# aszepieniec/stark-brainfuck

Hardware: AMD Instinct MI355X
Metric: goldilocks_ntt_field_elements_per_sec (higher is better)
Workload: dtype u64 (mod 2^64-2^32+1)

## Files before the change

include/bfstark.h:

```cpp
#ifndef BFSTARK_H
#define BFSTARK_H

#include <stddef.h>
#include <stdint.h>

#ifdef __cplusplus
extern "C" {
#endif

enum {
    BFS_OK = 0,
    BFS_ERR_NOT_POW2 = 1,
    BFS_ERR_NOT_ROOT = 2,
    BFS_ERR_NOT_PRIMITIVE = 3,
    BFS_ERR_TOO_MANY_COEFFS = 4,
    BFS_ERR_ZERO_IN_BATCH_INVERSE = 5,
    BFS_ERR_BAD_ARG = 6,
    BFS_ERR_HIP = 7,
    BFS_ERR_LENGTH = 8,
    BFS_ERR_TOO_MANY_INDICES = 9
};

int bfs_version(void);
const char* bfs_last_error(void);
int bfs_device_count(int* count);
int bfs_set_device(int device);
int bfs_malloc(void** d_ptr, size_t bytes);
int bfs_free(void* d_ptr);
int bfs_malloc_async(void** d_ptr, size_t bytes, void* stream);
int bfs_free_async(void* d_ptr, void* stream);
int bfs_pool_trim(void);
int bfs_pool_stats(size_t* live_bytes, size_t* cached_bytes);
int bfs_host_alloc(void** h_ptr, size_t bytes);
int bfs_host_free(void* h_ptr);
int bfs_memcpy_h2d(void* d_dst, const void* h_src, size_t bytes, void* stream);
int bfs_memcpy_d2h(void* h_dst, const void* d_src, size_t bytes, void* stream);
int bfs_memcpy_d2d(void* d_dst, const void* d_src, size_t bytes, void* stream);
int bfs_memset(void* d_dst, int value, size_t bytes, void* stream);
int bfs_stream_synchronize(void* stream);
int bfs_stream_create(void** stream);
int bfs_stream_destroy(void* stream);
int bfs_event_create(void** event);
int bfs_event_destroy(void* event);
int bfs_event_record(void* event, void* stream);
int bfs_event_elapsed_ms(void* start, void* stop, float* ms);

uint64_t bfs_gl_primitive_root(uint32_t log_n);
uint64_t bfs_gl_mul(uint64_t a, uint64_t b);
uint64_t bfs_gl_inv(uint64_t a);
uint64_t bfs_gl_pow(uint64_t a, uint64_t e);

int bfs_gl_ntt(const uint64_t* d_in, uint64_t n_in, uint64_t in_stride, uint64_t* d_out, uint64_t out_stride,
               uint32_t log_n, uint32_t batch, uint64_t root, uint64_t coset_shift, uint64_t post_scale,
               void* stream);

int bfs_ntt_tune(const uint64_t* d_in, uint64_t in_stride, uint64_t* d_out, uint64_t out_stride, uint32_t log_n, uint32_t batch, uint64_t root,
                 void* stream, int* route);
int bfs_ntt_route_forget(const void* d_ptr, size_t* forgotten);

int bfs_ntt_route_probe_info(float* us, int* route, unsigned long long* probes);

int bfs_gl_scale(const uint64_t* d_in, uint64_t* d_out, uint64_t n, uint64_t stride, uint32_t batch, uint64_t factor,
                 void* stream);

int bfs_gl_mul_pointwise(const uint64_t* d_a, const uint64_t* d_b, uint64_t* d_out, uint64_t n, void* stream);
int bfs_gl_batch_inverse(const uint64_t* d_in, uint64_t* d_out, uint64_t n, void* stream);
int bfs_xfe_mul_pointwise(const uint64_t* d_a, uint64_t a_stride, const uint64_t* d_b, uint64_t b_stride, uint64_t* d_out, uint64_t out_stride,
                          uint64_t n, void* stream);
int bfs_xfe_batch_inverse(const uint64_t* d_in, uint64_t in_stride, uint64_t* d_out, uint64_t out_stride, uint64_t n, void* stream);

typedef struct bfs_ptree bfs_ptree;
int bfs_ptree_build(const uint64_t* d_points, uint64_t n, void* stream, bfs_ptree** out);
uint64_t bfs_ptree_size(const bfs_ptree* tree);
int bfs_ptree_zerofier(const bfs_ptree* tree, uint64_t* d_out, void* stream);
int bfs_ptree_evaluate(const bfs_ptree* tree, const uint64_t* d_coeffs, uint64_t n_coeffs, uint64_t in_stride, uint32_t batch,
                       uint64_t* d_out, uint64_t out_stride, void* stream);
int bfs_ptree_interpolate(const bfs_ptree* tree, const uint64_t* d_values, uint64_t in_stride, uint32_t batch, uint64_t* d_out,
                          uint64_t out_stride, void* stream);
int bfs_ptree_free(bfs_ptree* tree, void* stream);

void* bfs_ps_new(void);
void bfs_ps_free(void* ps);
void* bfs_ps_loads(const uint8_t* data, size_t len);
uint64_t bfs_ps_obj_bytes(void* ps, const uint8_t* data, size_t len);
uint64_t bfs_ps_obj_int(void* ps, uint64_t value);
uint64_t bfs_ps_obj_xfe(void* ps, const uint64_t limbs[3]);
uint64_t bfs_ps_obj_bfe(void* ps, uint64_t value, int field_id);
uint64_t bfs_ps_obj_xfe_from(void* ps, const uint64_t* coefficient_handles, size_t n);
uint64_t bfs_ps_obj_list(void* ps, const uint64_t* handles, size_t n);
uint64_t bfs_ps_obj_tuple(void* ps, const uint64_t* handles, size_t n);
int bfs_ps_push(void* ps, uint64_t handle);
size_t bfs_ps_num_objects(void* ps);
uint64_t bfs_ps_object_at(void* ps, size_t index);
int bfs_ps_serialize(void* ps, size_t count, uint8_t* out, size_t capacity, size_t* length);
int bfs_ps_fiat_shamir(void* ps, size_t count, uint8_t* out, size_t num_bytes);
size_t bfs_ps_prefetch_fiat_shamir(void* ps, const size_t* counts, size_t n, size_t num_bytes);
int bfs_ps_merkle_verify(void* ps, uint64_t element_handle, uint64_t salt_handle, uint64_t path_handle, uint64_t index, const uint8_t* root,
                         size_t root_len, int* ok);
int bfs_xfe_inner_product(const uint64_t* weights, const uint64_t* terms, size_t count, uint64_t out[3]);
int bfs_ps_push_digest_fiat_shamir(void* ps, const uint8_t digest[64], uint8_t* out, size_t num_bytes);
int bfs_ps_push_digests_fiat_shamir(void* ps, const uint8_t* digests, size_t count, uint8_t* out, size_t num_bytes, int* used_lookahead);
int bfs_ps_obj_dumps(void* ps, uint64_t handle, uint8_t* out, size_t capacity, size_t* length);
int bfs_ps_obj_kind(void* ps, uint64_t handle);
size_t bfs_ps_obj_len(void* ps, uint64_t handle);
uint64_t bfs_ps_obj_item(void* ps, uint64_t handle, size_t i);
int bfs_ps_obj_get_bytes(void* ps, uint64_t handle, uint8_t* out, size_t capacity);
int bfs_ps_obj_get_limbs(void* ps, uint64_t handle, uint64_t limbs[3]);
int bfs_sample_weights(const uint8_t* randomness, size_t len, size_t count, uint64_t* out);
uint64_t bfs_gl_sample(const uint8_t* bytes, size_t len);
void bfs_xfe_sample(const uint8_t* bytes, size_t len, uint64_t out[3]);

typedef struct bfs_gather_request {
    const uint64_t* d_base;
    uint32_t nwords, stride;
    uint64_t out_offset;
} bfs_gather_request;
int bfs_gather(const bfs_gather_request* requests, uint32_t count, uint64_t* h_out, void* stream);
int bfs_stark_push_openings(void* ps, const bfs_gather_request* base_row, uint32_t n_base_req, int32_t base_field_id,
                            const bfs_gather_request* ext_row, uint32_t n_ext_req, const uint64_t* ext_moduli, uint32_t n_ext_cols,
                            uint64_t n, const uint8_t* d_base_nodes, const uint8_t* base_salts, int base_salts_on_device,
                            const uint8_t* d_ext_nodes, const uint8_t* ext_salts, int ext_salts_on_device,
                            const uint64_t* d_combination, uint64_t combination_stride, const uint8_t* d_combination_nodes,
                            const uint64_t* indices, uint32_t n_indices, const uint64_t* distances, uint32_t n_distances,
                            uint64_t* out_leaf_handles, void* stream);
int bfs_stark_push_openings_cosets(void* ps, const bfs_gather_request* base_row, uint32_t n_base_req, int32_t base_field_id,
                                   const bfs_gather_request* ext_row, uint32_t n_ext_req, const uint64_t* ext_moduli, uint32_t n_ext_cols,
                                   uint64_t n, const uint8_t* d_base_nodes, const uint8_t* base_salts, int base_salts_on_device,
                                   const uint8_t* d_ext_nodes, const uint8_t* ext_salts, int ext_salts_on_device,
                                   const uint64_t* d_combination, uint64_t combination_stride, const uint8_t* d_combination_nodes,
                                   uint32_t log2_coset, const uint64_t* indices, uint32_t n_indices, const uint64_t* distances,
                                   uint32_t n_distances, void* stream);

int bfs_merkle_build_xfe(const uint64_t* d_limbs, uint64_t limb_stride, uint64_t n, uint8_t* d_nodes, void* stream);
int bfs_merkle_build_bfe(const uint64_t* d_values, uint64_t n, uint8_t* d_nodes, void* stream);
int bfs_merkle_build_bytes(const uint8_t* d_data, const uint64_t* d_word_offsets, const uint32_t* d_lengths, uint64_t n,
                           uint8_t* d_nodes, void* stream);
int bfs_merkle_open(const uint8_t* d_nodes, uint32_t depth, uint64_t index, uint8_t* h_path, void* stream);
int bfs_merkle_build_xfe_cosets(const uint64_t* d_limbs, uint64_t limb_stride, uint64_t n, uint32_t log2_coset, uint8_t* d_nodes, void* stream);
uint64_t bfs_coset_trees_by_rows(void);
typedef struct bfs_row_column {
    const uint64_t* d_values;
    int32_t is_ext;
    int32_t field_id;
} bfs_row_column;
int bfs_merkle_build_rows_range(const bfs_row_column* columns, uint32_t ncols, uint64_t n, uint64_t limb_stride, const uint8_t* salts,
                                int salts_on_device, uint8_t* d_nodes, void* stream);
int bfs_merkle_build_rows(const bfs_row_column* columns, uint32_t ncols, uint64_t n, const uint8_t* salts, int salts_on_device,
                          uint8_t* d_nodes, void* stream);
int bfs_merkle_build_rows_root(const bfs_row_column* columns, uint32_t ncols, uint64_t n, uint64_t limb_stride, const uint8_t* salts,
                               int salts_on_device, uint8_t* d_nodes, uint8_t h_root[64], void* stream);
int bfs_row_template_steps(const bfs_row_column* columns, uint32_t ncols, uint32_t code, int salted, uint32_t out_header[4],
                           uint64_t* out_steps, uint32_t steps_cap, uint32_t* out_ints, uint32_t ints_cap, uint64_t* out_hash);
uint64_t bfs_row_generated_launches(void);
int bfs_random_fill(const uint8_t seed[32], uint64_t* d_out, uint64_t nwords, void* stream);
int bfs_xfe_sample_fill(const uint8_t seed[32], uint64_t* d_out, uint64_t count, uint64_t limb_stride, void* stream);

typedef struct bfs_trace_pad_table {
    const uint64_t* d_rows;
    uint64_t rows, row_stride, height;
    uint64_t* d_out;
    uint8_t *d_mask0, *d_mask1, *d_mask2;
    int32_t kind;
    uint32_t width;
} bfs_trace_pad_table;
int bfs_trace_pad(const bfs_trace_pad_table* tables, uint32_t count, void* stream);

int bfs_xfe_fold(const uint64_t* d_in, uint64_t in_stride, uint64_t* d_out, uint64_t out_stride, uint32_t log_n,
                 const uint64_t alpha[3], uint64_t offset, uint64_t omega, void* stream);
int bfs_xfe_fold_multi(const uint64_t* d_in, uint64_t in_stride, uint64_t* d_out, uint64_t out_stride, uint32_t log_n, uint32_t log2_folding,
                       const uint64_t alpha[3], uint64_t offset, uint64_t omega, void* stream);
void* bfs_fri_session_new(void);
void bfs_fri_session_free(void* session);
int bfs_fri_session_set_folding(void* session, uint32_t log2_folding);
int bfs_fri_session_set_coset_leaves(void* session, int on);
int bfs_fri_session_set_grinding(void* session, uint32_t bits, uint64_t window);
int bfs_pow_check(const uint8_t seed[32], uint32_t bits, uint64_t nonce, int* ok);
int bfs_pow_search(const uint8_t seed[32], uint32_t bits, uint64_t first_nonce, uint64_t count, uint64_t* nonce, int* found, void* stream);
int bfs_fri_commit(void* session, void* ps, const uint64_t* d_codeword, uint64_t limb_stride, uint32_t log_n, uint64_t offset,
                   uint64_t omega, uint32_t expansion_factor, void* stream);
int bfs_fri_query(void* session, void* ps, uint32_t num_colinearity_tests, uint64_t* h_top_level_indices, void* stream);
int bfs_fri_session_alias(void* session, void* ps, uint32_t round, uint64_t index, uint64_t element_handle);
int bfs_fri_session_round0_tree(void* session, const uint8_t* d_nodes, const uint8_t h_root[64]);
int bfs_fri_session_round0_coset_tree(void* session, const uint8_t* d_nodes, uint64_t num_leaves, const uint8_t h_root[64]);
int bfs_fri_prove(void* ps, const uint64_t* d_codeword, uint64_t limb_stride, uint32_t log_n, uint64_t offset, uint64_t omega,
                  uint32_t expansion_factor, uint32_t num_colinearity_tests, uint64_t* h_top_level_indices, void* stream);
int bfs_fri_prove_folded(void* ps, const uint64_t* d_codeword, uint64_t limb_stride, uint32_t log_n, uint64_t offset, uint64_t omega,
                         uint32_t expansion_factor, uint32_t log2_folding, uint32_t num_colinearity_tests, uint64_t* h_top_level_indices,
                         void* stream);
int bfs_fri_prove_cosets(void* ps, const uint64_t* d_codeword, uint64_t limb_stride, uint32_t log_n, uint64_t offset, uint64_t omega,
                         uint32_t expansion_factor, uint32_t log2_folding, int coset_leaves, uint32_t num_colinearity_tests,
                         uint64_t* h_top_level_indices, void* stream);
void bfs_fri_last_timing(double out[6]);
uint32_t bfs_fri_session_rounds(void* session);
uint64_t bfs_fri_session_round_leaves(void* session, uint32_t round);
int bfs_fri_session_round(void* session, uint32_t round, const uint64_t** d_codeword, uint64_t* length, uint64_t* limb_stride,
                          const uint8_t** d_nodes, uint8_t h_root[64]);

int bfs_selftest_field(uint32_t log_count, uint64_t* mismatches);
int bfs_selftest_field_pairs(const uint64_t* h_pairs, uint64_t n, uint64_t* h_out);

#define BFS_VM_DEFAULT_MAX_CYCLES (1ull << 24)
int bfs_vm_trace_new(const uint64_t* program, size_t n_words, const uint32_t* input, size_t n_input, uint64_t max_cycles, void** trace);
void bfs_vm_trace_free(void* trace);
int bfs_vm_trace_size(void* trace, int which, size_t* words);
int bfs_vm_trace_copy(void* trace, int which, uint64_t* out);

int bfs_xfe_scan(int kind, const uint64_t* x1, const uint64_t* x2, const uint64_t* x3, const uint8_t* mask, uint64_t n,
                 const uint64_t constants[12], const uint64_t initial[3], int record_before, uint64_t* out, uint64_t terminal[3]);
int bfs_host_transpose(const uint64_t* src, size_t rows, size_t src_stride, size_t width, uint64_t* dst, size_t dst_stride);
int bfs_xfe_scan_device(int kind, const uint64_t* d_x1, const uint64_t* d_x2, const uint64_t* d_x3, uint64_t shift1,
                        const uint8_t* d_mask, uint64_t n, const uint64_t constants[12], const uint64_t initial[3],
                        int record_before, uint64_t* d_out, uint64_t out_stride, uint64_t* d_terminal, uint64_t* terminal, void* stream);
typedef struct bfs_scan_spec {
    int32_t kind, record_before;
    const uint64_t *d_x1, *d_x2, *d_x3;
    uint64_t shift1;
    const uint8_t* d_mask;
    uint64_t n;
    uint64_t constants[12];
    uint64_t initial[3];
    uint64_t* d_out;
    uint64_t out_stride;
    uint64_t* d_terminal;
} bfs_scan_spec;
int bfs_xfe_scan_device_many(const bfs_scan_spec* specs, uint32_t count, void* stream);

typedef struct bfs_comb_source {
    const uint64_t* ptr;
    uint32_t is_ext, pad;
    uint64_t shift;
    uint64_t wa[3], wb[3];
} bfs_comb_source;
int bfs_poly_support(const uint64_t* d_coeffs, uint64_t stride, uint64_t len, uint32_t batch, uint64_t* h_masks, void* stream);
int bfs_poly_randomize(uint64_t* d_coeffs, uint64_t stride, uint64_t h, uint32_t batch, uint64_t point, const uint64_t* h_values, void* stream);
int bfs_air_num_quotients(int table);
int bfs_air_counts(int table, int counts[3]);
int bfs_air_evaluate(int table, const uint64_t* base_row, const uint64_t* base_next, const uint64_t* ext_row, const uint64_t* ext_next,
                     const uint64_t* h_challenges, const uint64_t* h_terminals, const uint64_t* h_params, uint64_t* out);
typedef struct bfs_air_violation {
    uint64_t first_row;
    uint64_t count;
} bfs_air_violation;
int bfs_air_base_counts(int table, int counts[2]);
int bfs_air_check(int table, int extended, const uint64_t* d_base, const uint64_t* d_ext, uint64_t rows, uint64_t ld,
                  const uint64_t* h_challenges, const uint64_t* h_terminals, const uint64_t* h_params, bfs_air_violation* h_out, void* stream);
int bfs_air_quotients(int table, const uint64_t* d_base, const uint64_t* d_ext, uint64_t* d_out, uint32_t log_n, uint64_t unit_distance,
                      uint64_t height, uint64_t omicron_inv, uint64_t offset, uint64_t omega, const uint64_t* h_challenges,
                      const uint64_t* h_terminals, const uint64_t* h_params, void* stream);
int bfs_difference_quotient(const uint64_t* d_lhs, const uint64_t* d_rhs, uint64_t* d_out, uint32_t log_n, uint64_t offset, uint64_t omega, void* stream);
int bfs_combination(const bfs_comb_source* h_sources, uint32_t count, const uint64_t* d_randomizer, const uint64_t* h_randomizer_weight,
                    uint64_t* d_out, uint32_t log_n, uint64_t offset, uint64_t omega, void* stream);

typedef struct bfs_comb_weight {
    uint64_t wa[3], wb[3];
    uint64_t shift;
} bfs_comb_weight;
int bfs_air_combine(int table, const uint64_t* d_base, const uint64_t* d_ext, uint32_t log_n, uint64_t unit_distance, uint64_t height,
                    uint64_t omicron_inv, uint64_t offset, uint64_t omega, const uint64_t* h_challenges, const uint64_t* h_terminals,
                    const uint64_t* h_params, const bfs_comb_weight* h_weights, const uint64_t* d_randomizer,
                    const uint64_t* h_randomizer_weight, uint64_t* d_acc, const uint64_t* const* d_zerofier_inverses, void* stream);
int bfs_difference_combine(const uint64_t* d_lhs, const uint64_t* d_rhs, uint32_t log_n, uint64_t offset, uint64_t omega,
                           const bfs_comb_weight* h_weight, uint64_t* d_acc, const uint64_t* d_inv_x_minus_1, void* stream);
int bfs_zerofier_inverses(uint32_t log_n, uint64_t offset, uint64_t omega, uint32_t count, const uint32_t* h_is_power, const uint64_t* h_values,
                          uint64_t* d_out, void* stream);
int bfs_air_combine_rows(int table, const uint64_t* d_base, const uint64_t* d_ext, uint32_t log_n, uint64_t unit_distance, uint64_t height,
                         uint64_t omicron_inv, uint64_t offset, uint64_t omega, const uint64_t* h_challenges, const uint64_t* h_terminals,
                         const uint64_t* h_params, const bfs_comb_weight* h_weights, const uint64_t* d_randomizer,
                         const uint64_t* h_randomizer_weight, uint64_t* d_acc, const uint64_t* const* d_zerofier_inverses, uint64_t first_row,
                         uint64_t num_rows, void* stream);
int bfs_difference_combine_rows(const uint64_t* d_lhs, const uint64_t* d_rhs, uint32_t log_n, uint64_t offset, uint64_t omega,
                                const bfs_comb_weight* h_weight, uint64_t* d_acc, const uint64_t* d_inv_x_minus_1, uint64_t first_row,
                                uint64_t num_rows, void* stream);
int bfs_zerofier_inverses_rows(uint32_t log_n, uint64_t offset, uint64_t omega, uint32_t count, const uint32_t* h_is_power, const uint64_t* h_values,
                               uint64_t* d_out, uint64_t first_row, uint64_t num_rows, void* stream);

typedef struct bfs_stark_params {
    uint32_t log_n;
    uint32_t expansion_factor, num_colinearity_checks, security_level;
    uint64_t offset, omega;
    uint64_t max_degree;
    uint64_t heights[3];
} bfs_stark_params;
typedef struct bfs_stark_table_in {
    const uint64_t* values;
    uint64_t rows, row_stride;
} bfs_stark_table_in;
typedef struct bfs_stark_randomness {
    const uint8_t* randomizer_seed;
    const uint64_t* randomizer_limbs;
    const uint64_t* base_randomizers;
    const uint8_t* base_salt_seed;
    const uint8_t* base_salts;
    uint64_t initials[6];
    const uint64_t* ext_randomizers;
    const uint8_t* ext_salt_seed;
    const uint8_t* ext_salts;
} bfs_stark_randomness;
void* bfs_stark_session_new(void);
void bfs_stark_session_free(void* session);
int bfs_stark_session_set_fri(void* session, uint32_t log2_folding, int coset_leaves, uint32_t grinding_bits);
int bfs_stark_commit(void* session, void* ps, const bfs_stark_params* params, const bfs_stark_table_in* tables, const bfs_stark_randomness* randomness,
                     uint64_t* out_challenges, uint64_t* out_scan_terminals, uint64_t* out_io_terminals, double* out_ms, void* stream);
int bfs_stark_finish(void* session, void* ps, const uint64_t* terminal_handles, const uint64_t* terminals, const uint64_t* shifts,
                     uint32_t num_terms, int32_t base_field_id, const uint64_t* distances, uint32_t n_distances, uint64_t* out_indices,
                     uint8_t* out_weights_seed, uint64_t* out_fri_indices, double* out_ms, void* stream);

typedef struct bfs_stark_verify_params {
    uint32_t log_n, expansion_factor, num_colinearity_checks, security_level;
    uint64_t offset, omega;
    uint64_t heights[5], lengths[5], omicrons[5];
    uint32_t num_distances, pad;
    uint64_t distances[8];
    const uint64_t* program; size_t program_len;
    const uint64_t* input; size_t n_input;
    const uint64_t* output; size_t n_output;
} bfs_stark_verify_params;
int bfs_stark_verify_begin(void* ps, const bfs_stark_verify_params* params, uint64_t* out_challenges, uint64_t* out_terminals, int* verdict);
int bfs_stark_verify_finish(void* ps, const bfs_stark_verify_params* params, const uint64_t* shifts, uint32_t num_terms, int* verdict);
int bfs_stark_verify_finish_fri(void* ps, const bfs_stark_verify_params* params, const uint64_t* shifts, uint32_t num_terms, uint32_t log2_folding,
                                int coset_leaves, uint32_t grinding_bits, int* verdict);

#ifdef __cplusplus
}
#endif
#endif
```

stark_brainfuck_amd/_lib.py:

```python
import ctypes
import os

_HERE = os.path.dirname(os.path.abspath(__file__))
LIB_PATH = os.environ.get("BFS_LIB_PATH") or os.path.join(_HERE, "libbfstark_hip.so")

u64 = ctypes.c_uint64
u32 = ctypes.c_uint32
vp = ctypes.c_void_p
sz = ctypes.c_size_t
ci = ctypes.c_int

BFS_OK = 0
ASSERT_CODES = {1, 2, 3, 4, 5, 8, 9}

_SIGNATURES = {
    "bfs_version": (ci, []),
    "bfs_last_error": (ctypes.c_char_p, []),
    "bfs_device_count": (ci, [ctypes.POINTER(ci)]),
    "bfs_set_device": (ci, [ci]),
    "bfs_malloc": (ci, [ctypes.POINTER(vp), sz]),
    "bfs_free": (ci, [vp]),
    "bfs_malloc_async": (ci, [ctypes.POINTER(vp), sz, vp]),
    "bfs_free_async": (ci, [vp, vp]),
    "bfs_pool_trim": (ci, []),
    "bfs_pool_stats": (ci, [ctypes.POINTER(sz), ctypes.POINTER(sz)]),
    "bfs_host_alloc": (ci, [ctypes.POINTER(vp), sz]),
    "bfs_host_free": (ci, [vp]),
    "bfs_memcpy_h2d": (ci, [vp, vp, sz, vp]),
    "bfs_memcpy_d2h": (ci, [vp, vp, sz, vp]),
    "bfs_memcpy_d2d": (ci, [vp, vp, sz, vp]),
    "bfs_memset": (ci, [vp, ci, sz, vp]),
    "bfs_stream_synchronize": (ci, [vp]),
    "bfs_stream_create": (ci, [ctypes.POINTER(vp)]),
    "bfs_stream_destroy": (ci, [vp]),
    "bfs_event_create": (ci, [ctypes.POINTER(vp)]),
    "bfs_event_destroy": (ci, [vp]),
    "bfs_event_record": (ci, [vp, vp]),
    "bfs_event_elapsed_ms": (ci, [vp, vp, ctypes.POINTER(ctypes.c_float)]),
    "bfs_gl_primitive_root": (u64, [u32]),
    "bfs_gl_mul": (u64, [u64, u64]),
    "bfs_gl_inv": (u64, [u64]),
    "bfs_gl_pow": (u64, [u64, u64]),
    "bfs_gl_ntt": (ci, [vp, u64, u64, vp, u64, u32, u32, u64, u64, u64, vp]),
    "bfs_ntt_route_probe_info": (ci, [vp, vp, vp]),
    "bfs_ntt_tune": (ci, [vp, u64, vp, u64, u32, u32, u64, vp, ctypes.POINTER(ci)]),
    "bfs_ntt_route_forget": (ci, [vp, ctypes.POINTER(sz)]),
    "bfs_gl_scale": (ci, [vp, vp, u64, u64, u32, u64, vp]),
    "bfs_gl_mul_pointwise": (ci, [vp, vp, vp, u64, vp]),
    "bfs_gl_batch_inverse": (ci, [vp, vp, u64, vp]),
    "bfs_xfe_mul_pointwise": (ci, [vp, u64, vp, u64, vp, u64, u64, vp]),
    "bfs_xfe_batch_inverse": (ci, [vp, u64, vp, u64, u64, vp]),
    "bfs_ptree_build": (ci, [vp, u64, vp, ctypes.POINTER(vp)]),
    "bfs_ptree_size": (u64, [vp]),
    "bfs_ptree_zerofier": (ci, [vp, vp, vp]),
    "bfs_ptree_evaluate": (ci, [vp, vp, u64, u64, u32, vp, u64, vp]),
    "bfs_ptree_interpolate": (ci, [vp, vp, u64, u32, vp, u64, vp]),
    "bfs_ptree_free": (ci, [vp, vp]),
    "bfs_ps_new": (vp, []),
    "bfs_ps_loads": (vp, [ctypes.c_char_p, sz]),
    "bfs_ps_free": (None, [vp]),
    "bfs_ps_obj_bytes": (u64, [vp, ctypes.c_char_p, sz]),
    "bfs_ps_obj_int": (u64, [vp, u64]),
    "bfs_ps_obj_xfe": (u64, [vp, ctypes.POINTER(u64)]),
    "bfs_ps_obj_bfe": (u64, [vp, u64, ci]),
    "bfs_ps_obj_xfe_from": (u64, [vp, ctypes.POINTER(u64), sz]),
    "bfs_ps_obj_list": (u64, [vp, ctypes.POINTER(u64), sz]),
    "bfs_ps_obj_tuple": (u64, [vp, ctypes.POINTER(u64), sz]),
    "bfs_ps_push": (ci, [vp, u64]),
    "bfs_ps_num_objects": (sz, [vp]),
    "bfs_ps_object_at": (u64, [vp, sz]),
    "bfs_ps_serialize": (ci, [vp, sz, vp, sz, ctypes.POINTER(sz)]),
    "bfs_ps_prefetch_fiat_shamir": (sz, [vp, ctypes.POINTER(sz), sz, sz]),
    "bfs_ps_fiat_shamir": (ci, [vp, sz, vp, sz]),
    "bfs_sample_weights": (ci, [ctypes.c_char_p, sz, sz, ctypes.POINTER(u64)]),
    "bfs_ps_push_digest_fiat_shamir": (ci, [vp, ctypes.c_char_p, vp, sz]),
    "bfs_ps_push_digests_fiat_shamir": (ci, [vp, ctypes.c_char_p, sz, vp, sz, ctypes.POINTER(ci)]),
    "bfs_ps_obj_dumps": (ci, [vp, u64, vp, sz, ctypes.POINTER(sz)]),
    "bfs_ps_merkle_verify": (ci, [vp, u64, u64, u64, u64, ctypes.c_char_p, sz, ctypes.POINTER(ci)]),
    "bfs_xfe_inner_product": (ci, [ctypes.POINTER(u64), ctypes.POINTER(u64), sz, ctypes.POINTER(u64)]),
    "bfs_ps_obj_kind": (ci, [vp, u64]),
    "bfs_ps_obj_len": (sz, [vp, u64]),
    "bfs_ps_obj_item": (u64, [vp, u64, sz]),
    "bfs_ps_obj_get_bytes": (ci, [vp, u64, vp, sz]),
    "bfs_ps_obj_get_limbs": (ci, [vp, u64, ctypes.POINTER(u64)]),
    "bfs_gl_sample": (u64, [ctypes.c_char_p, sz]),
    "bfs_xfe_sample": (None, [ctypes.c_char_p, sz, ctypes.POINTER(u64)]),
    "bfs_gather": (ci, [vp, u32, vp, vp]),
    "bfs_merkle_build_xfe": (ci, [vp, u64, u64, vp, vp]),
    "bfs_merkle_build_xfe_cosets": (ci, [vp, u64, u64, u32, vp, vp]),
    "bfs_coset_trees_by_rows": (u64, []),
    "bfs_merkle_build_bfe": (ci, [vp, u64, vp, vp]),
    "bfs_merkle_build_bytes": (ci, [vp, vp, vp, u64, vp, vp]),
    "bfs_merkle_open": (ci, [vp, u32, u64, vp, vp]),
    "bfs_merkle_build_rows": (ci, [vp, u32, u64, vp, ci, vp, vp]),
    "bfs_stark_push_openings": (ci, [vp, vp, u32, ctypes.c_int32, vp, u32, ctypes.POINTER(u64), u32, u64, vp, vp, ci, vp, vp, ci, vp, u64, vp,
                                     ctypes.POINTER(u64), u32, ctypes.POINTER(u64), u32, ctypes.POINTER(u64), vp]),
    "bfs_stark_push_openings_cosets": (ci, [vp, vp, u32, ctypes.c_int32, vp, u32, ctypes.POINTER(u64), u32, u64, vp, vp, ci, vp, vp, ci, vp, u64, vp,
                                            u32, ctypes.POINTER(u64), u32, ctypes.POINTER(u64), u32, vp]),
    "bfs_merkle_build_rows_range": (ci, [vp, u32, u64, u64, vp, ci, vp, vp]),
    "bfs_merkle_build_rows_root": (ci, [vp, u32, u64, u64, vp, ci, vp, vp, vp]),
    "bfs_row_template_steps": (ci, [vp, u32, u32, ci, vp, vp, u32, vp, u32, vp]),
    "bfs_trace_pad": (ci, [vp, u32, vp]),
    "bfs_row_generated_launches": (u64, []),
    "bfs_random_fill": (ci, [ctypes.c_char_p, vp, u64, vp]),
    "bfs_xfe_sample_fill": (ci, [ctypes.c_char_p, vp, u64, u64, vp]),
    "bfs_xfe_fold": (ci, [vp, u64, vp, u64, u32, ctypes.POINTER(u64), u64, u64, vp]),
    "bfs_xfe_fold_multi": (ci, [vp, u64, vp, u64, u32, u32, ctypes.POINTER(u64), u64, u64, vp]),
    "bfs_fri_session_new": (vp, []),
    "bfs_fri_session_set_folding": (ci, [vp, u32]),
    "bfs_fri_session_set_coset_leaves": (ci, [vp, ci]),
    "bfs_fri_session_set_grinding": (ci, [vp, u32, u64]),
    "bfs_pow_check": (ci, [ctypes.c_char_p, u32, u64, ctypes.POINTER(ci)]),
    "bfs_pow_search": (ci, [ctypes.c_char_p, u32, u64, u64, ctypes.POINTER(u64), ctypes.POINTER(ci), vp]),
    "bfs_fri_session_round0_coset_tree": (ci, [vp, vp, u64, ctypes.c_char_p]),
    "bfs_fri_prove_cosets": (ci, [vp, vp, u64, u32, u64, u64, u32, u32, ci, u32, ctypes.POINTER(u64), vp]),
    "bfs_fri_session_round_leaves": (u64, [vp, u32]),
    "bfs_fri_session_free": (None, [vp]),
    "bfs_fri_commit": (ci, [vp, vp, vp, u64, u32, u64, u64, u32, vp]),
    "bfs_fri_query": (ci, [vp, vp, u32, ctypes.POINTER(u64), vp]),
    "bfs_fri_session_alias": (ci, [vp, vp, u32, u64, u64]),
    "bfs_fri_session_round0_tree": (ci, [vp, vp, ctypes.c_char_p]),
    "bfs_fri_prove": (ci, [vp, vp, u64, u32, u64, u64, u32, u32, ctypes.POINTER(u64), vp]),
    "bfs_fri_prove_folded": (ci, [vp, vp, u64, u32, u64, u64, u32, u32, u32, ctypes.POINTER(u64), vp]),
    "bfs_fri_last_timing": (None, [ctypes.POINTER(ctypes.c_double)]),
    "bfs_fri_session_rounds": (u32, [vp]),
    "bfs_fri_session_round": (ci, [vp, u32, ctypes.POINTER(vp), ctypes.POINTER(u64), ctypes.POINTER(u64), ctypes.POINTER(vp), vp]),
    "bfs_selftest_field": (ci, [u32, ctypes.POINTER(u64)]),
    "bfs_selftest_field_pairs": (ci, [vp, u64, vp]),
    "bfs_vm_trace_new": (ci, [ctypes.POINTER(u64), sz, ctypes.POINTER(u32), sz, u64, ctypes.POINTER(vp)]),
    "bfs_vm_trace_free": (None, [vp]),
    "bfs_vm_trace_size": (ci, [vp, ci, ctypes.POINTER(sz)]),
    "bfs_vm_trace_copy": (ci, [vp, ci, vp]),
    "bfs_xfe_scan": (ci, [ci, vp, vp, vp, vp, u64, ctypes.POINTER(u64), ctypes.POINTER(u64), ci, vp, ctypes.POINTER(u64)]),
    "bfs_xfe_scan_device_many": (ci, [vp, ctypes.c_uint32, vp]),
    "bfs_xfe_scan_device": (ci, [ci, vp, vp, vp, u64, vp, u64, ctypes.POINTER(u64), ctypes.POINTER(u64), ci, vp, u64, vp, ctypes.POINTER(u64), vp]),
    "bfs_poly_support": (ci, [vp, u64, u64, u32, ctypes.POINTER(u64), vp]),
    "bfs_poly_randomize": (ci, [vp, u64, u64, u32, u64, ctypes.POINTER(u64), vp]),
    "bfs_air_num_quotients": (ci, [ci]),
    "bfs_air_evaluate": (ci, [ci, ctypes.POINTER(u64), ctypes.POINTER(u64), ctypes.POINTER(u64), ctypes.POINTER(u64), ctypes.POINTER(u64),
                              ctypes.POINTER(u64), ctypes.POINTER(u64), ctypes.POINTER(u64)]),
    "bfs_air_quotients": (ci, [ci, vp, vp, vp, u32, u64, u64, u64, u64, u64, ctypes.POINTER(u64), ctypes.POINTER(u64), ctypes.POINTER(u64), vp]),
    "bfs_difference_quotient": (ci, [vp, vp, vp, u32, u64, u64, vp]),
    "bfs_combination": (ci, [vp, u32, vp, ctypes.POINTER(u64), vp, u32, u64, u64, vp]),
    "bfs_air_combine": (ci, [ci, vp, vp, u32, u64, u64, u64, u64, u64, ctypes.POINTER(u64), ctypes.POINTER(u64), ctypes.POINTER(u64), vp, vp,
                             ctypes.POINTER(u64), vp, ctypes.POINTER(vp), vp]),
    "bfs_difference_combine": (ci, [vp, vp, u32, u64, u64, vp, vp, vp, vp]),
    "bfs_zerofier_inverses": (ci, [u32, u64, u64, u32, ctypes.POINTER(u32), ctypes.POINTER(u64), vp, vp]),
    "bfs_host_transpose": (ci, [vp, sz, sz, sz, vp, sz]),
    "bfs_air_combine_rows": (ci, [ci, vp, vp, u32, u64, u64, u64, u64, u64, ctypes.POINTER(u64), ctypes.POINTER(u64), ctypes.POINTER(u64), vp, vp,
                                  ctypes.POINTER(u64), vp, ctypes.POINTER(vp), u64, u64, vp]),
    "bfs_difference_combine_rows": (ci, [vp, vp, u32, u64, u64, vp, vp, vp, u64, u64, vp]),
    "bfs_zerofier_inverses_rows": (ci, [u32, u64, u64, u32, ctypes.POINTER(u32), ctypes.POINTER(u64), vp, u64, u64, vp]),
    "bfs_air_counts": (ci, [ci, ctypes.POINTER(ci)]),
    "bfs_air_base_counts": (ci, [ci, ctypes.POINTER(ci)]),
    "bfs_air_check": (ci, [ci, ci, vp, vp, u64, u64, ctypes.POINTER(u64), ctypes.POINTER(u64), ctypes.POINTER(u64), vp, vp]),
    "bfs_stark_verify_begin": (ci, [vp, vp, ctypes.POINTER(u64), ctypes.POINTER(u64), ctypes.POINTER(ci)]),
    "bfs_stark_verify_finish": (ci, [vp, vp, ctypes.POINTER(u64), u32, ctypes.POINTER(ci)]),
    "bfs_stark_verify_finish_fri": (ci, [vp, vp, ctypes.POINTER(u64), u32, u32, ci, u32, ctypes.POINTER(ci)]),
    "bfs_stark_session_set_fri": (ci, [vp, u32, ci, u32]),
    "bfs_stark_session_new": (vp, []),
    "bfs_stark_session_free": (None, [vp]),
    "bfs_stark_commit": (ci, [vp, vp, vp, vp, vp, ctypes.POINTER(u64), ctypes.POINTER(u64), ctypes.POINTER(u64), ctypes.POINTER(ctypes.c_double), vp]),
    "bfs_stark_finish": (ci, [vp, vp, ctypes.POINTER(u64), ctypes.POINTER(u64), ctypes.POINTER(u64), u32, ctypes.c_int32, ctypes.POINTER(u64), u32,
                              ctypes.POINTER(u64), vp, ctypes.POINTER(u64), ctypes.POINTER(ctypes.c_double), vp]),
}

_EXT_SIGNATURES = {
    "bfs_poly_eval_points": (ci, [vp, u64, u64, u32, ctypes.POINTER(u64), u32, vp, vp]),
    "bfs_deep_quotient": (ci, [vp, u32, u64, u32, u64, u64, ctypes.POINTER(u64), ctypes.POINTER(u64), u32, ctypes.POINTER(u64), vp, u64, vp]),
}

_OPEN_SIGNATURES = {
    "bfsx_poly_eval_columns": (ci, [vp, u32, ctypes.POINTER(u64), u32, vp, vp]),
    "bfsx_deep_quotient_groups": (ci, [vp, u32, u64, u32, u64, u64, ctypes.POINTER(u32), ctypes.POINTER(u32), u32, ctypes.POINTER(u64), u32,
                                       ctypes.POINTER(u32), ctypes.POINTER(u64), ctypes.POINTER(u64), vp, u64, vp]),
}

_ROUNDS_SIGNATURES = {
    "bfsr_deep_quotient_rounds": (ci, [vp, u32, u64, u32, u64, u64, ctypes.POINTER(u32), ctypes.POINTER(u32), u32, ctypes.POINTER(u64), u32,
                                       ctypes.POINTER(u32), ctypes.POINTER(u64), ctypes.POINTER(u64), vp, u64, ctypes.POINTER(u32), vp]),
}


class GatherRequest(ctypes.Structure):
    _fields_ = [("d_base", vp), ("nwords", u32), ("stride", u32), ("out_offset", u64)]


class AirViolation(ctypes.Structure):
    _fields_ = [("first_row", u64), ("count", u64)]


class RowColumn(ctypes.Structure):
    _fields_ = [("d_values", vp), ("is_ext", ctypes.c_int32), ("field_id", ctypes.c_int32)]


class EvalColumn(ctypes.Structure):
    _fields_ = [("d_coeffs", vp), ("n_coeffs", u64)]


class TracePadTable(ctypes.Structure):
    _fields_ = [("d_rows", vp), ("rows", u64), ("row_stride", u64), ("height", u64), ("d_out", vp), ("d_mask0", vp), ("d_mask1", vp),
                ("d_mask2", vp), ("kind", ctypes.c_int32), ("width", u32)]


class CombSource(ctypes.Structure):
    _fields_ = [("ptr", vp), ("is_ext", u32), ("pad", u32), ("shift", u64), ("wa", u64 * 3), ("wb", u64 * 3)]

class ScanSpec(ctypes.Structure):
    _fields_ = [("kind", ctypes.c_int32), ("record_before", ctypes.c_int32), ("d_x1", vp), ("d_x2", vp), ("d_x3", vp), ("shift1", u64),
                ("d_mask", vp), ("n", u64), ("constants", u64 * 12), ("initial", u64 * 3), ("d_out", vp), ("out_stride", u64),
                ("d_terminal", vp)]


class StarkParams(ctypes.Structure):
    _fields_ = [("log_n", u32), ("expansion_factor", u32), ("num_colinearity_checks", u32), ("security_level", u32), ("offset", u64),
                ("omega", u64), ("max_degree", u64), ("heights", u64 * 3)]


class StarkVerifyParams(ctypes.Structure):
    _fields_ = [("log_n", u32), ("expansion_factor", u32), ("num_colinearity_checks", u32), ("security_level", u32), ("offset", u64),
                ("omega", u64), ("heights", u64 * 5), ("lengths", u64 * 5), ("omicrons", u64 * 5), ("num_distances", u32), ("pad", u32),
                ("distances", u64 * 8), ("program", vp), ("program_len", sz), ("input", vp), ("n_input", sz), ("output", vp), ("n_output", sz)]


class StarkTableIn(ctypes.Structure):
    _fields_ = [("values", vp), ("rows", u64), ("row_stride", u64)]


class StarkRandomness(ctypes.Structure):
    _fields_ = [("randomizer_seed", vp), ("randomizer_limbs", vp), ("base_randomizers", vp), ("base_salt_seed", vp), ("base_salts", vp),
                ("initials", u64 * 6), ("ext_randomizers", vp), ("ext_salt_seed", vp), ("ext_salts", vp)]


class CombWeight(ctypes.Structure):
    _fields_ = [("wa", u64 * 3), ("wb", u64 * 3), ("shift", u64)]


_lib = None


class BackendUnavailable(RuntimeError):
    pass


def exported_symbols():
    return sorted(_SIGNATURES)


def ext_exported_symbols():
    return sorted(_EXT_SIGNATURES)


def open_exported_symbols():
    return sorted(_OPEN_SIGNATURES)


def rounds_exported_symbols():
    return sorted(_ROUNDS_SIGNATURES)


def load():
    global _lib
    if _lib is not None:
        return _lib
    if not os.path.exists(LIB_PATH):
        raise BackendUnavailable(
            "libbfstark_hip.so is not built (%s). Run `python -m stark_brainfuck_amd.build`; "
            "there is no CPU fallback for the hot path." % LIB_PATH)
    try:
        import torch
    except ImportError:
        pass
    lib = ctypes.CDLL(LIB_PATH)
    for name, (res, args) in list(_SIGNATURES.items()) + list(_EXT_SIGNATURES.items()) + list(_OPEN_SIGNATURES.items()) + list(_ROUNDS_SIGNATURES.items()):
        fn = getattr(lib, name)
        fn.restype = res
        fn.argtypes = args
    _lib = lib
    return lib


def check(rc):
    if rc == BFS_OK:
        return
    msg = load().bfs_last_error().decode("utf-8", "replace")
    if rc in ASSERT_CODES:
        raise AssertionError(msg)
    raise RuntimeError("libbfstark_hip: error %d: %s" % (rc, msg))
```

stark_brainfuck_amd/csrc/coset.hip:

```cpp
#include <atomic>
#include <vector>

#include "../../include/bfstark.h"
#include "coset_core.hpp"
#include "runtime.hpp"

namespace bfs {

constexpr u32 COSET_THREADS = 64;

template <int K, int A>
__global__ void __launch_bounds__(COSET_THREADS) coset_leaves_kernel(FriFoldArgs f, u64* cw, u64 cw_stride, u64 q, u64* leaf_digests,
                                                                     const u64* block0_states, u64* not_mine, u64 token) {
    typedef CosetShape<A> Shape;
    __shared__ __attribute__((aligned(16))) unsigned char blk[COSET_LANE_BYTES * COSET_THREADS];
    unsigned char* const buf = blk + COSET_LANE_BYTES * threadIdx.x;
    const u64 c = (u64)blockIdx.x * COSET_THREADS + threadIdx.x;
    bool ok = c < q;
    u32 int_bytes = 0;
    if (ok) {
#pragma nounroll
        for (u32 m = 0; m < (u32)A; ++m) {
            const u64 at = c + (u64)m * q;
            u64 c0, c1, c2;
            if constexpr (K > 0) {
                const Xfe r = fri_fold_point<K>(f, at);
                c0 = r.c[0]; c1 = r.c[1]; c2 = r.c[2];
                cw[at] = c0; cw[cw_stride + at] = c1; cw[2 * cw_stride + at] = c2;
            } else {
                c0 = cw[at]; c1 = cw[cw_stride + at]; c2 = cw[2 * cw_stride + at];
            }
            int_bytes += pickle_int_len(c0) + pickle_int_len(c1) + pickle_int_len(c2);
            ok = ok && c2 != 0;
        }
        if (!ok) __hip_atomic_store(not_mine, token, __ATOMIC_RELAXED, __HIP_MEMORY_SCOPE_SYSTEM);
    }
    CosetLane s;
    s.pos = 0; s.consumed = 128; s.total = Shape::CONST_BYTES + int_bytes;
    u64 x0 = 0, x1 = 0, x2 = 0;
    if (ok) {
        const u64* ms = block0_states + (size_t)(int_bytes - Shape::MIN_INT_BYTES) * 8;
#pragma unroll
        for (int j = 0; j < 8; ++j) s.h[j] = ms[j];
        x0 = cw[c]; x1 = cw[cw_stride + c]; x2 = cw[2 * cw_stride + c];
    }
    u32 stage = 0;
    bool done = false;
    while (true) {
        stage = (u32)__builtin_amdgcn_readfirstlane(stage);
        const bool behind = __any(ok && s.pos < 128);
        bool want;
        if (!done) want = ok && coset_lane_ready(s) && (s.pos > COSET_FORCE || !behind);
        else want = ok && s.consumed < s.total;
        if (__any(want)) {
            if (want) coset_compress(s, buf, done);
            continue;
        }
        if (done) break;
        if (ok) {
            coset_stage<A>(s, buf, stage, x0, x1, x2);
            if (stage >= 2 && stage + 1 < Shape::STAGES) {
                const u64 at = c + (u64)(stage - 1) * q;
                x0 = cw[at]; x1 = cw[cw_stride + at]; x2 = cw[2 * cw_stride + at];
            }
        }
        ++stage;
        done = stage == Shape::STAGES;
    }
    if (!ok) return;
    u64* out = leaf_digests + c * 8;
#pragma unroll
    for (int j = 0; j < 8; ++j) out[j] = s.h[j];
}

template <int A>
static int coset_block0_states(const u64** d_table) {
    constexpr u64 KEY = 0x636F736574ULL;
    if (cached_table_lookup(KEY, A, 0, d_table)) return BFS_OK;
    std::vector<u64> host((size_t)CosetShape<A>::BLOCK0_STATES * 8);
    for (u32 e = 0; e < CosetShape<A>::BLOCK0_STATES; ++e) {
        unsigned char block[128];
        coset_block0<A>(CosetShape<A>::MIN_INT_BYTES + e, block);
        u64 m[16], st[8];
        memcpy(m, block, 128);
        blake2b_init(st);
        blake2b_compress(st, m, 128, false);
        memcpy(&host[(size_t)e * 8], st, 64);
    }
    return cached_table(KEY, A, 0, host.data(), host.size(), d_table);
}

template <int KF, int A = 1 << KF>
static int coset_leaves_launch_a(const FriFoldArgs* fold, u64* d_cw, u64 cw_stride, u64 q, u64* d_leaf_digests, hipStream_t stream, u64* not_mine, u64 token) {
    const u64* d_states = nullptr;
    BFS_TRY(coset_block0_states<A>(&d_states));
    const dim3 grid((u32)((q + COSET_THREADS - 1) / COSET_THREADS)), block(COSET_THREADS);
    if (fold != nullptr) hipLaunchKernelGGL((coset_leaves_kernel<KF, A>), grid, block, 0, stream, *fold, d_cw, cw_stride, q, d_leaf_digests, d_states, not_mine, token);
    else hipLaunchKernelGGL((coset_leaves_kernel<0, A>), grid, block, 0, stream, FriFoldArgs{}, d_cw, cw_stride, q, d_leaf_digests, d_states, not_mine, token);
    BFS_HIP(hipGetLastError());
    return BFS_OK;
}

int coset_tree_launch(const FriFoldArgs* fold, u64* d_cw, u64 cw_stride, u64 q, u32 log2_coset, u64* d_nodes, hipStream_t stream, u64* not_mine,
                      u64 token, u64* root_out, u64 seq) {
    if (q == 0 || (q & (q - 1))) { set_error("internal: coset tree over %llu leaves", (unsigned long long)q); return BFS_ERR_BAD_ARG; }
    if (fold != nullptr && (fold->log2_folding != log2_coset || fold->half != (q << log2_coset))) { set_error("internal: coset tree and fold disagree"); return BFS_ERR_BAD_ARG; }
    BFS_TRY(with_fold_factor(log2_coset, [&](auto k) -> int {
        return coset_leaves_launch_a<decltype(k)::value>(fold, d_cw, cw_stride, q, d_nodes + q * 8, stream, not_mine, token);
    }));
    return merkle_inner_launch(d_nodes, tree_depth(q), q, stream, root_out, seq);
}

static std::atomic<u64> g_coset_trees_by_rows{0};

int coset_tree_rows(const u64* d_cw, u64 cw_stride, u64 q, u32 log2_coset, u64* d_nodes, unsigned char h_root[64], hipStream_t stream) {
    bfs_row_column cols[8];
    const u32 a = 1u << log2_coset;
    g_coset_trees_by_rows.fetch_add(1, std::memory_order_relaxed);
    for (u32 m = 0; m < a; ++m) cols[m] = bfs_row_column{d_cw + (u64)m * q, 1, 0};
    return bfs_merkle_build_rows_root(cols, a, q, cw_stride, nullptr, 0, (uint8_t*)d_nodes, h_root, stream);
}

}

using namespace bfs;

extern "C" uint64_t bfs_coset_trees_by_rows(void) { return g_coset_trees_by_rows.load(std::memory_order_relaxed); }

extern "C" int bfs_merkle_build_xfe_cosets(const uint64_t* d_limbs, uint64_t limb_stride, uint64_t n, uint32_t log2_coset, uint8_t* d_nodes, void* stream_) {
    hipStream_t stream = (hipStream_t)stream_;
    if (((uintptr_t)d_nodes & 15) != 0) { set_error("d_nodes must be 16-byte aligned"); return BFS_ERR_BAD_ARG; }
    if (log2_coset < 1 || log2_coset > 3) { set_error("bfs_merkle_build_xfe_cosets: log2_coset must be 1, 2 or 3 (got %u)", log2_coset); return BFS_ERR_BAD_ARG; }
    if (n == 0 || (n & (n - 1)) || (n >> log2_coset) == 0) { set_error("bfs_merkle_build_xfe_cosets: n must be a power of two, at least the coset size"); return BFS_ERR_BAD_ARG; }
    if (limb_stride < n) { set_error("bfs_merkle_build_xfe_cosets: limb_stride < n"); return BFS_ERR_BAD_ARG; }
    PinnedLease flag;
    BFS_TRY(flag.get(64));
    volatile u64* seen = (volatile u64*)flag.host;
    *seen = 0;
    const u64 q = n >> log2_coset;
    BFS_TRY(coset_tree_launch(nullptr, (u64*)d_limbs, limb_stride, q, log2_coset, (u64*)d_nodes, stream, (u64*)flag.dev, 1, nullptr, 0));
    BFS_HIP(hipStreamSynchronize(stream));
    if (*seen == 0) return BFS_OK;
    return coset_tree_rows(d_limbs, limb_stride, q, log2_coset, (u64*)d_nodes, nullptr, stream);
}
```

stark_brainfuck_amd/csrc/fri.hip:

```cpp
#include <algorithm>
#include <chrono>
#include <map>
#include <unordered_map>
#include <vector>

#include "../../include/bfstark.h"
#include "blake2b.hpp"
#include "refpickle.hpp"
#include "runtime.hpp"

namespace bfs {

template <int K>
__global__ void __launch_bounds__(K == 1 ? 1024 : 256) fri_fold_kernel(FriFoldArgs f, u64* out, u64 out_stride) {
    for (u64 i = (u64)blockIdx.x * blockDim.x + threadIdx.x; i < f.half; i += (u64)gridDim.x * blockDim.x) {
        const Xfe r = fri_fold_point<K>(f, i);
        out[i] = r.c[0];
        out[out_stride + i] = r.c[1];
        out[2 * out_stride + i] = r.c[2];
    }
}

constexpr u32 FRI_FOLD_GRID_MAX = 4096;
static int fri_fold_launch(const FriFoldArgs& f, u64* out, u64 out_stride, hipStream_t stream) {
    u32 grid = (u32)((f.half + 255) / 256);
    if (grid > FRI_FOLD_GRID_MAX) grid = FRI_FOLD_GRID_MAX;
    return with_fold_factor(f.log2_folding, [&](auto k) -> int {
        hipLaunchKernelGGL(fri_fold_kernel<decltype(k)::value>, dim3(grid), dim3(256), 0, stream, f, out, out_stride);
        BFS_HIP(hipGetLastError());
        return BFS_OK;
    });
}

struct GatherReq {
    const u64* base;
    u32 nwords, stride;
    u64 out_offset;
};
__global__ void gather_requests_kernel(const GatherReq* req, u32 count, u64* out) {
    for (u32 i = blockIdx.x * blockDim.x + threadIdx.x; i < count; i += gridDim.x * blockDim.x) {
        const GatherReq r = req[i];
        for (u32 w = 0; w < r.nwords; ++w) out[r.out_offset + w] = r.base[(u64)w * r.stride];
    }
}

static int gather_run(const std::vector<GatherReq>& reqs, u64 nwords, hipStream_t stream, PinnedLease& req_area, PinnedLease& res_area, const u64** words) {
    BFS_TRY(req_area.get(reqs.size() * sizeof(GatherReq)));
    BFS_TRY(res_area.get(nwords * sizeof(u64)));
    memcpy(req_area.host, reqs.data(), reqs.size() * sizeof(GatherReq));
    hipLaunchKernelGGL(gather_requests_kernel, dim3((u32)((reqs.size() + 255) / 256)), dim3(256), 0, stream, (const GatherReq*)req_area.dev, (u32)reqs.size(),
                       (u64*)res_area.dev);
    BFS_HIP(hipGetLastError());
    BFS_HIP(hipStreamSynchronize(stream));
    *words = (const u64*)res_area.host;
    return BFS_OK;
}

static thread_local double g_fri_timing[8] = {0, 0, 0, 0, 0, 0, 0, 0};
static inline double now_ms() { return std::chrono::duration<double, std::milli>(std::chrono::steady_clock::now().time_since_epoch()).count(); }

enum class TreePath : unsigned char {
    Borrowed,
    Coset,
    OneLaunch,
    FoldInLeaves,
    Codeword,
    SingleElement,
};

struct FriRound {
    const u64* cw = nullptr;
    u64 stride = 0, length = 0;
    u64 leaves = 0;
    u64* nodes = nullptr;
    TreePath path = TreePath::Codeword;
    unsigned char root[64];
};

struct RootMailbox {
    u64* host = nullptr;
    u64* dev = nullptr;
    u64 seq = 0;
    int init() {
        if (host) return BFS_OK;
        BFS_TRY(host_alloc(16 * sizeof(u64), (void**)&host));
        memset(host, 0, 16 * sizeof(u64));
        BFS_HIP(hipHostGetDevicePointer((void**)&dev, host, 0));
        return BFS_OK;
    }
    ~RootMailbox() { if (host) (void)host_release(host); }
};

struct FriSession {
    std::vector<FriRound> rounds;
    void* block = nullptr;
    bool use_workspace = false;
    RootMailbox mailbox;
    u32 log_n = 0;
    u32 log2_folding = 1;
    bool coset_leaves = false;
    u32 grinding_bits = 0;
    u64 grinding_window = POW_DEFAULT_WINDOW;
    u64 round0_leaves = 0;
    struct Key {
        u64 v;
        Key(u32 round, u64 index) : v(((u64)round << 48) | index) {}
        bool operator==(const Key& o) const { return v == o.v; }
    };
    struct KeyMap {
        std::vector<u64> keys;
        std::vector<u32> slots;
        std::vector<rp::Ref> vals;
        void reserve(size_t n) { size_t cap = 64; while (cap < 2 * n) cap <<= 1; if (cap > keys.size()) rehash(cap); vals.reserve(n); }
        void rehash(size_t cap) {
            std::vector<u64> k2(cap, 0);
            std::vector<u32> s2(cap, 0);
            for (size_t i = 0; i < keys.size(); ++i)
                if (keys[i]) { size_t j = slot_of(keys[i], cap); while (k2[j]) j = (j + 1) & (cap - 1); k2[j] = keys[i]; s2[j] = slots[i]; }
            keys.swap(k2); slots.swap(s2);
        }
        static size_t slot_of(u64 stored, size_t cap) { return (size_t)((stored * 0x9E3779B97F4A7C15ULL) >> 20) & (cap - 1); }
        size_t find(const Key& key) const {
            size_t j = slot_of(key.v + 1, keys.size());
            while (keys[j] && keys[j] != key.v + 1) j = (j + 1) & (keys.size() - 1);
            return j;
        }
        bool count(const Key& key) const { return !keys.empty() && keys[find(key)] != 0; }
        rp::Ref& operator[](const Key& key) {
            if (2 * (vals.size() + 1) > keys.size()) rehash(keys.empty() ? 64 : 2 * keys.size());
            const size_t j = find(key);
            if (!keys[j]) { keys[j] = key.v + 1; slots[j] = (u32)vals.size(); vals.emplace_back(); }
            return vals[slots[j]];
        }
    };
    KeyMap elements, nodes;
    std::vector<uint64_t> last_handles;
    hipStream_t block_stream = nullptr;
    const u64* round0_nodes = nullptr;
    unsigned char round0_root[64];
    ~FriSession() { if (block) (void)device_release(block, block_stream); }
};

static u32 fri_num_rounds(u64 length, u32 expansion, u32 k = 1) {
    u32 r = 0;
    while (length > expansion) { length /= 2; ++r; }
    return r == 0 ? 0 : (r - 1) / k + 1;
}

static int plan_rounds(FriSession& S, const u64* d_cw, u64 stride, u32 log_n, u64 omega, u32 expansion, hipStream_t stream) {
    const u64 N = 1ull << log_n;
    const u32 k = S.log2_folding;
    const u32 R = fri_num_rounds(N, expansion, k);
    if (k > 1 && R < 2) { set_error("cannot fold by %u with less than one fold", 1u << k); return BFS_ERR_BAD_ARG; }
    if (R < 1) { set_error("cannot do FRI with less than one round"); return BFS_ERR_BAD_ARG; }
    if (gl_pow(omega, N) != 1 || (log_n && gl_pow(omega, N / 2) == 1)) {
        set_error("error in commit: omega does not have the right order!");
        return BFS_ERR_NOT_ROOT;
    }
    S.log_n = log_n;
    S.rounds.assign(R, FriRound());
    const bool coset = S.coset_leaves;
    if (coset && R < 2) { set_error("cannot commit to cosets with less than one fold"); return BFS_ERR_BAD_ARG; }
    if (S.round0_nodes && S.round0_leaves != (coset ? N >> k : 0)) {
        set_error("the round-0 tree handed to the session has %llu leaves, this session's has %llu", (unsigned long long)(S.round0_leaves ? S.round0_leaves : N),
                  (unsigned long long)(coset ? N >> k : N));
        return BFS_ERR_BAD_ARG;
    }
    size_t words = 0;
    for (u32 r = 0; r < R; ++r) {
        FriRound& fr = S.rounds[r];
        const bool coset_round = coset && r + 1 < R;
        fr.length = N >> (k * r);
        fr.leaves = coset_round ? fr.length >> k : fr.length;
        fr.path = r == 0 && S.round0_nodes ? TreePath::Borrowed
                  : coset_round            ? TreePath::Coset
                  : fr.length < 2          ? TreePath::SingleElement
                  : fr.length <= FRI_FUSED_MAX ? TreePath::OneLaunch
                  : r >= 1                 ? TreePath::FoldInLeaves
                                           : TreePath::Codeword;
        words += (size_t)16 * fr.leaves + (r ? (size_t)3 * fr.length : 0);
    }
    u64* p = nullptr;
    if (S.use_workspace) {
        void* w = nullptr;
        BFS_TRY(workspace(4, words * sizeof(u64), stream, &w));
        p = (u64*)w;
    } else {
        if (S.block) { (void)device_release(S.block, S.block_stream); S.block = nullptr; }
        BFS_TRY(device_alloc(words * sizeof(u64), stream, &S.block));
        S.block_stream = stream;
        p = (u64*)S.block;
    }
    for (u32 r = 0; r < R; ++r) {
        FriRound& fr = S.rounds[r];
        fr.nodes = p; p += 16 * fr.leaves;
        if (r == 0) { fr.cw = d_cw; fr.stride = stride; }
        else { fr.cw = p; fr.stride = fr.length; p += 3 * fr.length; }
    }
    return S.mailbox.init();
}

static int launch_round_tree(FriSession& S, u32 r, const FriFoldArgs& fold, hipStream_t stream, u64* seq) {
    FriRound& fr = S.rounds[r];
    const bool folds = fold.in != nullptr;
    u64* const cw = (u64*)fr.cw;
    u64* const box = S.mailbox.dev;
    *seq = 0;
    if (folds != (r >= 1)) { set_error("internal: round %u of the plan and its fold disagree", r); return BFS_ERR_BAD_ARG; }
    switch (fr.path) {
    case TreePath::Borrowed:
        fr.nodes = (u64*)S.round0_nodes;
        memcpy(fr.root, S.round0_root, 64);
        return BFS_OK;
    case TreePath::SingleElement:
        if (folds) BFS_TRY(fri_fold_launch(fold, cw, fr.stride, stream));
        return merkle_build_xfe_launch(fr.cw, fr.stride, fr.length, fr.nodes, stream);
    case TreePath::Coset:
        *seq = ++S.mailbox.seq;
        return coset_tree_launch(folds ? &fold : nullptr, cw, fr.stride, fr.leaves, S.log2_folding, fr.nodes, stream, box + 9, *seq, box, *seq);
    case TreePath::OneLaunch:
        *seq = ++S.mailbox.seq;
        return fri_round_fused_launch(fold, cw, fr.stride, fr.length, fr.nodes, stream, box, *seq);
    case TreePath::FoldInLeaves:
        *seq = ++S.mailbox.seq;
        return merkle_build_xfe_fold_launch(fold, cw, fr.stride, fr.length, fr.nodes, stream, box, *seq);
    case TreePath::Codeword:
        *seq = ++S.mailbox.seq;
        return merkle_build_xfe_launch(fr.cw, fr.stride, fr.length, fr.nodes, stream, box, *seq);
    }
    set_error("internal: round %u has no tree path", r);
    return BFS_ERR_BAD_ARG;
}

int fri_commit(FriSession& S, rp::Transcript& ps, const u64* d_cw, u64 stride, u32 log_n, u64 offset, u64 omega,
               u32 expansion, hipStream_t stream) {
    const double t_begin = now_ms();
    BFS_TRY(plan_rounds(S, d_cw, stride, log_n, omega, expansion, stream));
    const u32 k = S.log2_folding;
    const u32 R = (u32)S.rounds.size();
    const u64 *winv_lo = nullptr, *winv_hi = nullptr;
    u32 lo_bits = 0;
    BFS_TRY(ntt_power_tables(gl_inv(omega), log_n, &winv_lo, &winv_hi, &lo_bits));
    u64 g = offset, w = omega;
    FriFoldArgs fold{};
    rp::Transcript::Lookahead look;
    static const bool lookahead_on = getenv("BFS_FRI_LOOKAHEAD") == nullptr || atoi(getenv("BFS_FRI_LOOKAHEAD")) != 0;
    static const bool trace = getenv("BFS_FRI_TRACE") != nullptr;
    bool looking = false, look_begun = false;
    auto begin_lookahead = [&]() {
        if (look_begun) return;
        look_begun = true;
        const double t_look = trace ? now_ms() : 0;
        looking = lookahead_on && R >= 3 && ps.lookahead_begin(look, R - 2);
        if (trace) fprintf(stderr, "fri look-ahead %s: %.1f us, %zu objects in front\n", looking ? "on" : "off", 1e3 * (now_ms() - t_look), ps.objects.size());
    };
    for (u32 r = 0; r < R; ++r) {
        FriRound& fr = S.rounds[r];
        unsigned char seed[32];
        bool have_seed = false, speculating = false;
        const double t_round = trace ? now_ms() : 0;
        double t_launched = 0, t_absorbed = 0, t_root = 0;
        rp::Transcript::Speculation speculation;
        auto await_root = [&](u64 seq) -> int {
            if (trace) t_launched = now_ms();
            if (r >= 1) begin_lookahead();
            if (r + 1 < R) {
                if (r == 0) { ps.fiat_shamir(ps.objects.size(), seed, 32); have_seed = true; }
                else if (!looking) { ps.speculate(speculation); speculating = true; }
            }
            if (trace) t_absorbed = now_ms();
            volatile u64* flag = S.mailbox.host + 8;
            u64 spins = 0;
            while (__atomic_load_n(flag, __ATOMIC_ACQUIRE) != seq) {
                if (++spins > (1ull << 22)) {
                    BFS_HIP(hipStreamSynchronize(stream));
                    if (__atomic_load_n(flag, __ATOMIC_ACQUIRE) != seq) { set_error("root mailbox was not written"); return BFS_ERR_HIP; }
                    break;
                }
            }
            memcpy(fr.root, S.mailbox.host, 64);
            return BFS_OK;
        };
        u64 seq = 0;
        BFS_TRY(launch_round_tree(S, r, fold, stream, &seq));
        if (seq != 0) {
            BFS_TRY(await_root(seq));
            if (fr.path == TreePath::Coset && __atomic_load_n(S.mailbox.host + 9, __ATOMIC_ACQUIRE) == seq) {
                BFS_TRY(coset_tree_rows(fr.cw, fr.stride, fr.leaves, k, fr.nodes, fr.root, stream));
            }
        } else if (fr.path == TreePath::SingleElement) {
            if (r >= 1) begin_lookahead();
            BFS_HIP(hipMemcpyAsync(fr.root, fr.nodes + 8, 64, hipMemcpyDeviceToHost, stream));
            BFS_HIP(hipStreamSynchronize(stream));
        }
        if (trace) t_root = now_ms();
        if (speculating) ps.resolve(speculation, fr.root, seed, 32);
        else if (r > 0 && looking) { ps.lookahead_next(look, fr.root, r + 1 < R ? seed : nullptr, 32); have_seed = r + 1 < R; }
        else if (r > 0) ps.objects.push_back(rp::mk_bytes(fr.root, 64));
        if (trace)
            fprintf(stderr, "fri round %2u  n %8llu  launch %6.1f us  absorb %6.1f us  wait %6.1f us  finish %6.1f us\n", r, (unsigned long long)fr.length,
                    1e3 * (t_launched - t_round), 1e3 * (t_absorbed - t_launched), 1e3 * (t_root - t_absorbed), 1e3 * (now_ms() - t_root));
        if (r == R - 1) break;
        if (!speculating && !have_seed) ps.fiat_shamir(ps.objects.size(), seed, 32);
        fold.in = fr.cw; fold.in_stride = fr.stride;
        fold.winv_lo = winv_lo; fold.winv_hi = winv_hi; fold.lo_bits = lo_bits; fold.round_shift = k * r;
        fri_fold_constants(fold, k, fr.length, rp::sample_xfe(seed, 32), g, w);
        for (u32 j = 0; j < k; ++j) { g = gl_sqr(g); w = gl_sqr(w); }
    }
    g_fri_timing[0] = now_ms() - t_begin;
    FriRound& last = S.rounds[R - 1];
    std::vector<u64> host(3 * last.length);
    if (last.stride == last.length) {
        BFS_HIP(hipMemcpyAsync(host.data(), last.cw, 3 * last.length * sizeof(u64), hipMemcpyDeviceToHost, stream));
    } else {
        for (int k = 0; k < 3; ++k)
            BFS_HIP(hipMemcpyAsync(host.data() + k * last.length, last.cw + k * last.stride, last.length * sizeof(u64), hipMemcpyDeviceToHost, stream));
    }
    BFS_HIP(hipStreamSynchronize(stream));
    std::vector<rp::Ref> items;
    for (u64 j = 0; j < last.length; ++j) {
        u64 l[3] = {host[j], host[last.length + j], host[2 * last.length + j]};
        rp::Ref e = ps.world.xfe_compact(l);
        S.elements[FriSession::Key(R - 1, j)] = e;
        items.push_back(e);
    }
    ps.objects.push_back(rp::mk_list(items));
    g_fri_timing[1] = now_ms() - t_begin - g_fri_timing[0];
    return BFS_OK;
}

static int sample_indices(const unsigned char seed[32], u64 size, u64 reduced_size, u32 number, std::vector<u64>& out) {
    if (number > reduced_size) {
        set_error("cannot sample more indices than available in last codeword; requested: %u, available: %llu", number, (unsigned long long)reduced_size);
        return BFS_ERR_TOO_MANY_INDICES;
    }
    out.clear();
    std::vector<u64> reduced;
    std::vector<unsigned char> msg(seed, seed + 32);
    while (out.size() < number) {
        unsigned char digest[64];
        blake2b_host(msg.data(), msg.size(), digest);
        msg.push_back(0);
        u128 acc = 0;
        for (int i = 0; i < 64; ++i) acc = ((acc << 8) | digest[i]) % size;
        u64 index = (u64)acc, red = index % reduced_size;
        bool seen = false;
        for (u64 x : reduced) seen |= (x == red);
        if (!seen) { out.push_back(index); reduced.push_back(red); }
    }
    return BFS_OK;
}

static int fri_grind(const FriSession& S, const unsigned char seed[32], hipStream_t stream, rp::Transcript& ps) {
    u64 words[4];
    memcpy(words, seed, 32);
    const u64 limit = 1ULL << (S.grinding_bits + 6);
    for (u64 first = 0; first < limit;) {
        const u64 count = limit - first < S.grinding_window ? limit - first : S.grinding_window;
        u64 nonce = 0;
        bool found = false;
        BFS_TRY(pow_search(words, S.grinding_bits, first, count, &nonce, &found, stream));
        if (found) { ps.objects.push_back(rp::mk_int(nonce)); return BFS_OK; }
        first += count;
    }
    set_error("bfs_fri_query: no nonce of %u grinding bits among the first 2^%u", S.grinding_bits, S.grinding_bits + 6);
    return BFS_ERR_BAD_ARG;
}

int fri_query(FriSession& S, rp::Transcript& ps, u32 t, u64* h_top, hipStream_t stream) {
    const u32 R = (u32)S.rounds.size();
    if (R < 2) { set_error("Fri.prove needs at least two rounds (fri.py:186 indexes codewords[1])"); return BFS_ERR_BAD_ARG; }
    const double t_begin = now_ms();
    unsigned char seed[32];
    ps.fiat_shamir(ps.objects.size(), seed, 32);
    if (S.grinding_bits) {
        BFS_TRY(fri_grind(S, seed, stream, ps));
        ps.fiat_shamir(ps.objects.size(), seed, 32);
    }
    std::vector<u64> top;
    BFS_TRY(sample_indices(seed, S.rounds[1].length, S.rounds[R - 1].length, t, top));
    for (u32 s = 0; s < t; ++s) h_top[s] = top[s];

    g_fri_timing[2] = now_ms() - t_begin;
    typedef FriSession::Key Key;
    const u32 fan = 1u << S.log2_folding;
    const bool coset = S.coset_leaves;
    {
        size_t depth_sum = 0;
        for (u32 r = 0; r < R; ++r) depth_sum += 64 - (size_t)__builtin_clzll(S.rounds[r].length);
        S.elements.reserve(S.elements.vals.size() + (size_t)(fan + 1) * t * R + 8);
        S.nodes.reserve((size_t)(fan + 1) * t * depth_sum / 2 + 64);
    }
    struct Opening {
        enum Kind : u32 { Element, TupleEnd , Path } kind;
        u32 round;
        u64 index;
    };
    std::vector<Opening> plan;
    plan.reserve((size_t)2 * (fan + 1) * t * (R - 1));
    for (u32 i = 0; i + 1 < R; ++i) {
        const u64 q = S.rounds[i + 1].length;
        for (u32 s = 0; s < t; ++s) {
            const u64 c = top[s] % q;
            for (u32 m = 0; m < fan; ++m) plan.push_back({Opening::Element, i, c + m * q});
            if (!coset) plan.push_back({Opening::Element, i + 1, c});
            plan.back().kind = Opening::TupleEnd;
        }
        for (u32 s = 0; s < t; ++s) {
            const u64 c = top[s] % q;
            if (coset) { plan.push_back({Opening::Path, i, c}); continue; }
            for (u32 m = 0; m < fan; ++m) plan.push_back({Opening::Path, i, c + m * q});
            if (i + 2 < R) plan.push_back({Opening::Path, i + 1, c});
        }
    }
    std::vector<GatherReq> reqs;
    std::vector<std::pair<int, Key>> order;
    reqs.reserve(4096); order.reserve(4096);
    u64 nwords = 0;
    auto need_element = [&](u32 r, u64 j) {
        Key key(r, j);
        if (S.elements.count(key)) return;
        S.elements[key] = rp::Ref();
        order.push_back({0, key});
        const FriRound& fr = S.rounds[r];
        reqs.push_back(GatherReq{fr.cw + j, 3u, (u32)fr.stride, nwords});
        nwords += 3;
    };
    auto need_path = [&](u32 r, u64 leaf) {
        const FriRound& fr = S.rounds[r];
        for (u64 k = fr.leaves | leaf; k > 1; k >>= 1) {
            Key key(r, k ^ 1);
            if (S.nodes.count(key)) continue;
            S.nodes[key] = rp::Ref();
            order.push_back({1, key});
            reqs.push_back(GatherReq{fr.nodes + (k ^ 1) * 8, 8u, 1u, nwords});
            nwords += 8;
        }
    };
    for (const Opening& o : plan) {
        if (o.kind == Opening::Path) need_path(o.round, o.index);
        else need_element(o.round, o.index);
    }
    g_fri_timing[3] = now_ms() - t_begin - g_fri_timing[2];
    const double t_gather = now_ms();
    const u64* words = nullptr;
    PinnedLease req_area, res_area;
    if (!reqs.empty()) BFS_TRY(gather_run(reqs, nwords, stream, req_area, res_area, &words));
    g_fri_timing[4] = now_ms() - t_gather;
    const double t_build = now_ms();
    size_t pos = 0;
    for (auto& o : order) {
        if (o.first == 0) {
            u64 l[3] = {words[pos], words[pos + 1], words[pos + 2]};
            pos += 3;
            S.elements[o.second] = ps.world.xfe_compact(l);
        } else {
            S.nodes[o.second] = rp::mk_bytes(words + pos, 64);
            pos += 8;
        }
    }
    auto path_obj = [&](u32 r, u64 leaf) {
        std::vector<rp::Ref> items;
        items.reserve(64 - (size_t)__builtin_clzll(S.rounds[r].leaves));
        for (u64 k = S.rounds[r].leaves | leaf; k > 1; k >>= 1) items.push_back(S.nodes[Key(r, k ^ 1)]);
        return rp::mk_list(std::move(items));
    };
    std::vector<rp::Ref> items;
    items.reserve(fan + 1);
    for (const Opening& o : plan) {
        if (o.kind == Opening::Path) { ps.objects.push_back(path_obj(o.round, o.index)); continue; }
        items.push_back(S.elements[Key(o.round, o.index)]);
        if (o.kind == Opening::TupleEnd) { ps.objects.push_back(rp::mk_tuple(items)); items.clear(); }
    }
    g_fri_timing[5] = now_ms() - t_build;
    return BFS_OK;
}

}

using namespace bfs;

extern "C" {

void* bfs_fri_session_new(void) { return new FriSession(); }
void bfs_fri_session_free(void* s) { delete (FriSession*)s; }

int bfs_fri_commit(void* session, void* ps, const uint64_t* d_codeword, uint64_t limb_stride, uint32_t log_n, uint64_t offset,
                   uint64_t omega, uint32_t expansion_factor, void* stream) {
    return fri_commit(*(FriSession*)session, *(rp::Transcript*)ps, d_codeword, limb_stride, log_n, offset, omega, expansion_factor, (hipStream_t)stream);
}

int bfs_fri_query(void* session, void* ps, uint32_t num_colinearity_tests, uint64_t* h_top_level_indices, void* stream) {
    return fri_query(*(FriSession*)session, *(rp::Transcript*)ps, num_colinearity_tests, h_top_level_indices, (hipStream_t)stream);
}

int bfs_fri_session_set_folding(void* session, uint32_t log2_folding) {
    FriSession* S = (FriSession*)session;
    if (log2_folding < 1 || log2_folding > 3) { set_error("bfs_fri_session_set_folding: log2_folding must be 1, 2 or 3 (got %u)", log2_folding); return BFS_ERR_BAD_ARG; }
    if (!S->rounds.empty()) { set_error("bfs_fri_session_set_folding: the session has already committed"); return BFS_ERR_BAD_ARG; }
    S->log2_folding = log2_folding;
    return BFS_OK;
}

int bfs_fri_session_set_coset_leaves(void* session, int on) {
    FriSession* S = (FriSession*)session;
    if (!S->rounds.empty()) { set_error("bfs_fri_session_set_coset_leaves: the session has already committed"); return BFS_ERR_BAD_ARG; }
    S->coset_leaves = on != 0;
    return BFS_OK;
}

int bfs_fri_session_set_grinding(void* session, uint32_t bits, uint64_t window) {
    FriSession* S = (FriSession*)session;
    if (bits > 40) { set_error("bfs_fri_session_set_grinding: bits must be in 0..40 (got %u)", bits); return BFS_ERR_BAD_ARG; }
    if (!S->rounds.empty()) { set_error("bfs_fri_session_set_grinding: the session has already committed"); return BFS_ERR_BAD_ARG; }
    S->grinding_bits = bits;
    S->grinding_window = window ? window : POW_DEFAULT_WINDOW;
    return BFS_OK;
}

static int fri_prove_run(void* ps, const uint64_t* d_codeword, uint64_t limb_stride, uint32_t log_n, uint64_t offset, uint64_t omega, uint32_t expansion_factor,
                         uint32_t log2_folding, int coset_leaves, uint32_t num_colinearity_tests, uint64_t* h_top_level_indices, void* stream) {
    FriSession S;
    S.use_workspace = true;
    BFS_TRY(bfs_fri_session_set_folding(&S, log2_folding));
    BFS_TRY(bfs_fri_session_set_coset_leaves(&S, coset_leaves));
    BFS_TRY(fri_commit(S, *(rp::Transcript*)ps, d_codeword, limb_stride, log_n, offset, omega, expansion_factor, (hipStream_t)stream));
    return fri_query(S, *(rp::Transcript*)ps, num_colinearity_tests, h_top_level_indices, (hipStream_t)stream);
}

int bfs_fri_prove(void* ps, const uint64_t* d_codeword, uint64_t limb_stride, uint32_t log_n, uint64_t offset, uint64_t omega,
                  uint32_t expansion_factor, uint32_t num_colinearity_tests, uint64_t* h_top_level_indices, void* stream) {
    return fri_prove_run(ps, d_codeword, limb_stride, log_n, offset, omega, expansion_factor, 1, 0, num_colinearity_tests, h_top_level_indices, stream);
}

int bfs_fri_prove_folded(void* ps, const uint64_t* d_codeword, uint64_t limb_stride, uint32_t log_n, uint64_t offset, uint64_t omega,
                         uint32_t expansion_factor, uint32_t log2_folding, uint32_t num_colinearity_tests, uint64_t* h_top_level_indices,
                         void* stream) {
    return fri_prove_run(ps, d_codeword, limb_stride, log_n, offset, omega, expansion_factor, log2_folding, 0, num_colinearity_tests, h_top_level_indices, stream);
}

int bfs_fri_prove_cosets(void* ps, const uint64_t* d_codeword, uint64_t limb_stride, uint32_t log_n, uint64_t offset, uint64_t omega,
                         uint32_t expansion_factor, uint32_t log2_folding, int coset_leaves, uint32_t num_colinearity_tests,
                         uint64_t* h_top_level_indices, void* stream) {
    return fri_prove_run(ps, d_codeword, limb_stride, log_n, offset, omega, expansion_factor, log2_folding, coset_leaves, num_colinearity_tests,
                         h_top_level_indices, stream);
}

static int stark_push_openings(void* ps_, const bfs_gather_request* base_row, uint32_t n_base_req, int32_t base_field_id,
                               const bfs_gather_request* ext_row, uint32_t n_ext_req, const uint64_t* ext_moduli, uint32_t n_ext_cols,
                               uint64_t n, const uint8_t* d_base_nodes, const uint8_t* base_salts, int base_salts_on_device,
                               const uint8_t* d_ext_nodes, const uint8_t* ext_salts, int ext_salts_on_device,
                               const uint64_t* d_combination, uint64_t combination_stride, const uint8_t* d_combination_nodes,
                               uint32_t log2_coset, const uint64_t* indices, uint32_t n_indices, const uint64_t* distances,
                               uint32_t n_distances, uint64_t* out_leaf_handles, void* stream_) {
    hipStream_t stream = (hipStream_t)stream_;
    rp::Transcript& ps = *(rp::Transcript*)ps_;
    if (n == 0 || (n & (n - 1))) { set_error("bfs_stark_push_openings: n must be a power of two"); return BFS_ERR_BAD_ARG; }
    if (log2_coset > 3 || (log2_coset && (n >> log2_coset) < 2)) { set_error("bfs_stark_push_openings_cosets: cosets of 2^%u in a codeword of %llu", log2_coset, (unsigned long long)n); return BFS_ERR_BAD_ARG; }
    if (combination_stride < n || combination_stride >> 32) { set_error("bfs_stark_push_openings: combination stride"); return BFS_ERR_BAD_ARG; }
    const u32 fan = 1u << log2_coset;
    const u64 comb_leaves = n >> log2_coset;
    u32 base_words = 0, ext_words = 0;
    for (u32 k = 0; k < n_base_req; ++k) base_words += base_row[k].nwords;
    for (u32 k = 0; k < n_ext_req; ++k) ext_words += ext_row[k].nwords;
    if (base_words < 3 || ext_words != 3 * n_ext_cols) { set_error("bfs_stark_push_openings: row layout"); return BFS_ERR_BAD_ARG; }
    std::vector<u64> rows, uniq_idx;
    for (u32 a = 0; a < n_indices; ++a) {
        for (u32 b = 0; b < n_distances; ++b) {
            const u64 r = (indices[a] + distances[b]) % n;
            if (std::find(rows.begin(), rows.end(), r) == rows.end()) rows.push_back(r);
        }
        if (indices[a] >= n) { set_error("bfs_stark_push_openings: index %llu outside the domain", (unsigned long long)indices[a]); return BFS_ERR_BAD_ARG; }
        const u64 leaf = indices[a] & (comb_leaves - 1);
        if (std::find(uniq_idx.begin(), uniq_idx.end(), leaf) == uniq_idx.end()) uniq_idx.push_back(leaf);
    }
    std::vector<GatherReq> reqs;
    u64 nwords = 0;
    auto want = [&](const u64* base, u32 words, u32 stride) { reqs.push_back(GatherReq{base, words, stride, nwords}); const u64 at = nwords; nwords += words; return at; };
    struct RowAt { u64 base, ext, base_salt, ext_salt; };
    std::vector<RowAt> row_at(rows.size());
    typedef FriSession::Key Key;
    FriSession::KeyMap node_at[3];
    std::vector<std::pair<int, u64>> node_list;
    std::vector<u64> node_off;
    const uint8_t* tree_nodes[3] = {d_base_nodes, d_ext_nodes, d_combination_nodes};
    const u64 tree_leaves[3] = {n, n, comb_leaves};
    auto want_path = [&](int tree, u64 leaf) {
        for (u64 k = tree_leaves[tree] | leaf; k > 1; k >>= 1) {
            const Key key(0, k ^ 1);
            if (node_at[tree].count(key)) continue;
            node_at[tree][key] = rp::mk_int(node_off.size());
            node_list.push_back({tree, k ^ 1});
            node_off.push_back(want((const u64*)(tree_nodes[tree] + 64 * (k ^ 1)), 8, 1));
        }
    };
    for (size_t r = 0; r < rows.size(); ++r) {
        const u64 i = rows[r];
        row_at[r].base = nwords;
        for (u32 k = 0; k < n_base_req; ++k) want(base_row[k].d_base + i, base_row[k].nwords, base_row[k].stride);
        row_at[r].ext = nwords;
        for (u32 k = 0; k < n_ext_req; ++k) want(ext_row[k].d_base + i, ext_row[k].nwords, ext_row[k].stride);
        row_at[r].base_salt = base_salts_on_device ? want((const u64*)(base_salts + 24 * i), 3, 1) : 0;
        row_at[r].ext_salt = ext_salts_on_device ? want((const u64*)(ext_salts + 24 * i), 3, 1) : 0;
        want_path(0, i);
        want_path(1, i);
    }
    std::vector<u64> leaf_at(uniq_idx.size());
    for (size_t a = 0; a < uniq_idx.size(); ++a) {
        leaf_at[a] = nwords;
        for (u32 j = 0; j < fan; ++j) want(d_combination + uniq_idx[a] + j * comb_leaves, 3, (u32)combination_stride);
        want_path(2, uniq_idx[a]);
    }
    PinnedLease req_area, res_area;
    const u64* words = nullptr;
    BFS_TRY(gather_run(reqs, nwords, stream, req_area, res_area, &words));
    std::vector<rp::Ref> node_obj(node_list.size());
    for (size_t k = 0; k < node_list.size(); ++k) node_obj[k] = rp::mk_bytes(words + node_off[k], 64);
    auto path_obj = [&](int tree, u64 leaf) {
        std::vector<rp::Ref> items;
        for (u64 k = tree_leaves[tree] | leaf; k > 1; k >>= 1) items.push_back(node_obj[node_at[tree][Key(0, k ^ 1)]->ival]);
        return rp::mk_list(items);
    };
    const rp::Ref base_field = ps.world.base_field(base_field_id);
    std::vector<rp::Ref> base_rows(rows.size()), ext_rows(rows.size()), base_salt_obj(rows.size()), ext_salt_obj(rows.size());
    std::vector<FriSession::KeyMap> shared(n_ext_cols);
    for (size_t r = 0; r < rows.size(); ++r) {
        const u64 i = rows[r];
        const u64* bw = words + row_at[r].base;
        std::vector<rp::Ref> items;
        u64 l[3] = {bw[0], bw[1], bw[2]};
        items.push_back(ps.world.xfe_compact(l));
        for (u32 k = 3; k < base_words; ++k) items.push_back(ps.world.bfe_in(bw[k], base_field));
        base_rows[r] = rp::mk_tuple(items);
        const u64* ew = words + row_at[r].ext;
        items.clear();
        for (u32 c = 0; c < n_ext_cols; ++c) {
            u64 e[3] = {ew[3 * c], ew[3 * c + 1], ew[3 * c + 2]};
            if (ext_moduli[c] == 0) { items.push_back(ps.world.xfe_compact(e)); continue; }
            const Key cls(0, i % ext_moduli[c]);
            if (!shared[c].count(cls)) {
                const int k = e[2] ? 3 : (e[1] ? 2 : (e[0] ? 1 : 0));
                std::vector<rp::Ref> coeffs;
                for (int j = 0; j < k; ++j) coeffs.push_back(ps.world.bfe(e[j], true));
                shared[c][cls] = rp::mk_list(coeffs);
            }
            items.push_back(ps.world.xfe_from(shared[c][cls]->items));
        }
        ext_rows[r] = rp::mk_tuple(items);
        base_salt_obj[r] = base_salts_on_device ? rp::mk_bytes(words + row_at[r].base_salt, 24) : rp::mk_bytes(base_salts + 24 * i, 24);
        ext_salt_obj[r] = ext_salts_on_device ? rp::mk_bytes(words + row_at[r].ext_salt, 24) : rp::mk_bytes(ext_salts + 24 * i, 24);
    }
    for (u32 a = 0; a < n_indices; ++a)
        for (u32 b = 0; b < n_distances; ++b) {
            const u64 i = (indices[a] + distances[b]) % n;
            const size_t r = (size_t)(std::find(rows.begin(), rows.end(), i) - rows.begin());
            ps.objects.push_back(base_rows[r]);
            ps.objects.push_back(rp::mk_tuple({base_salt_obj[r], path_obj(0, i)}));
            ps.objects.push_back(ext_rows[r]);
            ps.objects.push_back(rp::mk_tuple({ext_salt_obj[r], path_obj(1, i)}));
        }
    std::vector<rp::Ref> leaf_obj(uniq_idx.size());
    for (size_t a = 0; a < uniq_idx.size(); ++a) {
        std::vector<rp::Ref> items;
        for (u32 j = 0; j < fan; ++j) {
            const u64* w = words + leaf_at[a] + 3 * j;
            u64 l[3] = {w[0], w[1], w[2]};
            items.push_back(ps.world.xfe_compact(l));
        }
        leaf_obj[a] = log2_coset ? rp::mk_tuple(items) : items[0];
    }
    for (u32 a = 0; a < n_indices; ++a) {
        const u64 leaf = indices[a] & (comb_leaves - 1);
        const size_t u = (size_t)(std::find(uniq_idx.begin(), uniq_idx.end(), leaf) - uniq_idx.begin());
        ps.objects.push_back(leaf_obj[u]);
        ps.objects.push_back(path_obj(2, leaf));
        if (out_leaf_handles) out_leaf_handles[a] = ps.add(leaf_obj[u]);
    }
    return BFS_OK;
}

int bfs_stark_push_openings(void* ps, const bfs_gather_request* base_row, uint32_t n_base_req, int32_t base_field_id,
                            const bfs_gather_request* ext_row, uint32_t n_ext_req, const uint64_t* ext_moduli, uint32_t n_ext_cols,
                            uint64_t n, const uint8_t* d_base_nodes, const uint8_t* base_salts, int base_salts_on_device,
                            const uint8_t* d_ext_nodes, const uint8_t* ext_salts, int ext_salts_on_device,
                            const uint64_t* d_combination, uint64_t combination_stride, const uint8_t* d_combination_nodes,
                            const uint64_t* indices, uint32_t n_indices, const uint64_t* distances, uint32_t n_distances,
                            uint64_t* out_leaf_handles, void* stream) {
    return stark_push_openings(ps, base_row, n_base_req, base_field_id, ext_row, n_ext_req, ext_moduli, n_ext_cols, n, d_base_nodes, base_salts,
                               base_salts_on_device, d_ext_nodes, ext_salts, ext_salts_on_device, d_combination, combination_stride,
                               d_combination_nodes, 0, indices, n_indices, distances, n_distances, out_leaf_handles, stream);
}

int bfs_stark_push_openings_cosets(void* ps, const bfs_gather_request* base_row, uint32_t n_base_req, int32_t base_field_id,
                                   const bfs_gather_request* ext_row, uint32_t n_ext_req, const uint64_t* ext_moduli, uint32_t n_ext_cols,
                                   uint64_t n, const uint8_t* d_base_nodes, const uint8_t* base_salts, int base_salts_on_device,
                                   const uint8_t* d_ext_nodes, const uint8_t* ext_salts, int ext_salts_on_device,
                                   const uint64_t* d_combination, uint64_t combination_stride, const uint8_t* d_combination_nodes,
                                   uint32_t log2_coset, const uint64_t* indices, uint32_t n_indices, const uint64_t* distances,
                                   uint32_t n_distances, void* stream) {
    if (log2_coset < 1) { set_error("bfs_stark_push_openings_cosets: log2_coset must be 1, 2 or 3 (got %u)", log2_coset); return BFS_ERR_BAD_ARG; }
    return stark_push_openings(ps, base_row, n_base_req, base_field_id, ext_row, n_ext_req, ext_moduli, n_ext_cols, n, d_base_nodes, base_salts,
                               base_salts_on_device, d_ext_nodes, ext_salts, ext_salts_on_device, d_combination, combination_stride,
                               d_combination_nodes, log2_coset, indices, n_indices, distances, n_distances, nullptr, stream);
}

int bfs_gather(const bfs_gather_request* requests, uint32_t count, uint64_t* h_out, void* stream_) {
    hipStream_t stream = (hipStream_t)stream_;
    if (count == 0) return BFS_OK;
    static_assert(sizeof(bfs_gather_request) == sizeof(GatherReq), "layout of bfs_gather_request");
    u64 nwords = 0;
    std::vector<GatherReq> reqs(count);
    for (uint32_t i = 0; i < count; ++i) {
        reqs[i] = GatherReq{requests[i].d_base, requests[i].nwords, requests[i].stride, nwords};
        nwords += requests[i].nwords;
    }
    PinnedLease req_area, res_area;
    const u64* words = nullptr;
    BFS_TRY(gather_run(reqs, nwords, stream, req_area, res_area, &words));
    memcpy(h_out, words, nwords * sizeof(u64));
    return BFS_OK;
}

static int session_round0_tree(FriSession* S, const uint8_t* d_nodes, uint64_t leaves, const uint8_t h_root[64]) {
    S->round0_nodes = (const u64*)d_nodes;
    S->round0_leaves = leaves;
    memcpy(S->round0_root, h_root, 64);
    return BFS_OK;
}

int bfs_fri_session_round0_tree(void* session, const uint8_t* d_nodes, const uint8_t h_root[64]) {
    return session_round0_tree((FriSession*)session, d_nodes, 0, h_root);
}

int bfs_fri_session_round0_coset_tree(void* session, const uint8_t* d_nodes, uint64_t num_leaves, const uint8_t h_root[64]) {
    if (num_leaves == 0 || (num_leaves & (num_leaves - 1))) { set_error("bfs_fri_session_round0_coset_tree: %llu leaves", (unsigned long long)num_leaves); return BFS_ERR_BAD_ARG; }
    return session_round0_tree((FriSession*)session, d_nodes, num_leaves, h_root);
}

int bfs_fri_session_alias(void* session, void* ps, uint32_t round, uint64_t index, uint64_t element_handle) {
    rp::Ref r = ((rp::Transcript*)ps)->get(element_handle);
    if (!r) { set_error("bfs_fri_session_alias: unknown object handle"); return BFS_ERR_BAD_ARG; }
    if (((FriSession*)session)->coset_leaves) {
        set_error("bfs_fri_session_alias: a session that commits to cosets opens whole cosets; the caller cannot hold elements of one it has not opened");
        return BFS_ERR_BAD_ARG;
    }
    ((FriSession*)session)->elements[FriSession::Key(round, index)] = r;
    return BFS_OK;
}

void bfs_fri_last_timing(double out[6]) { for (int i = 0; i < 6; ++i) out[i] = g_fri_timing[i]; }

uint32_t bfs_fri_session_rounds(void* session) { return (uint32_t)((FriSession*)session)->rounds.size(); }

int bfs_fri_session_round(void* session, uint32_t r, const uint64_t** d_codeword, uint64_t* length, uint64_t* limb_stride,
                          const uint8_t** d_nodes, uint8_t h_root[64]) {
    FriSession* S = (FriSession*)session;
    if (r >= S->rounds.size()) { set_error("round %u out of range", r); return BFS_ERR_BAD_ARG; }
    const FriRound& fr = S->rounds[r];
    *d_codeword = fr.cw; *length = fr.length; *limb_stride = fr.stride; *d_nodes = (const uint8_t*)fr.nodes;
    memcpy(h_root, fr.root, 64);
    return BFS_OK;
}

uint64_t bfs_fri_session_round_leaves(void* session, uint32_t r) {
    FriSession* S = (FriSession*)session;
    return r < S->rounds.size() ? S->rounds[r].leaves : 0;
}

static int xfe_fold_run(const uint64_t* d_in, uint64_t in_stride, uint64_t* d_out, uint64_t out_stride, uint32_t log_n, uint32_t log2_folding,
                        const uint64_t alpha[3], uint64_t offset, uint64_t omega, void* stream) {
    const u64 N = 1ull << log_n;
    if (gl_pow(omega, N) != 1 || gl_pow(omega, N / 2) == 1) { set_error("error in commit: omega does not have the right order!"); return BFS_ERR_NOT_ROOT; }
    const u64 *lo = nullptr, *hi = nullptr;
    u32 lo_bits = 0;
    BFS_TRY(ntt_power_tables(gl_inv(omega), log_n, &lo, &hi, &lo_bits));
    Xfe a{{alpha[0] % GL_P, alpha[1] % GL_P, alpha[2] % GL_P}};
    FriFoldArgs f{};
    f.in = d_in; f.in_stride = in_stride;
    f.winv_lo = lo; f.winv_hi = hi; f.lo_bits = lo_bits; f.round_shift = 0;
    fri_fold_constants(f, log2_folding, N, a, offset % GL_P, omega);
    return fri_fold_launch(f, d_out, out_stride, (hipStream_t)stream);
}

int bfs_xfe_fold(const uint64_t* d_in, uint64_t in_stride, uint64_t* d_out, uint64_t out_stride, uint32_t log_n, const uint64_t alpha[3],
                 uint64_t offset, uint64_t omega, void* stream) {
    if (log_n == 0) { set_error("cannot fold a codeword of length 1"); return BFS_ERR_BAD_ARG; }
    return xfe_fold_run(d_in, in_stride, d_out, out_stride, log_n, 1, alpha, offset, omega, stream);
}

int bfs_xfe_fold_multi(const uint64_t* d_in, uint64_t in_stride, uint64_t* d_out, uint64_t out_stride, uint32_t log_n, uint32_t log2_folding,
                       const uint64_t alpha[3], uint64_t offset, uint64_t omega, void* stream) {
    const u64 N = 1ull << log_n;
    if (log2_folding < 1 || log2_folding > 3) { set_error("bfs_xfe_fold_multi: log2_folding must be 1, 2 or 3 (got %u)", log2_folding); return BFS_ERR_BAD_ARG; }
    if (log_n < log2_folding || log_n > 32) { set_error("cannot fold a codeword of length 2^%u by %u", log_n, 1u << log2_folding); return BFS_ERR_BAD_ARG; }
    if (in_stride < N || out_stride < (N >> log2_folding)) { set_error("bfs_xfe_fold_multi: a limb stride is shorter than its codeword"); return BFS_ERR_BAD_ARG; }
    return xfe_fold_run(d_in, in_stride, d_out, out_stride, log_n, log2_folding, alpha, offset, omega, stream);
}

}
```

stark_brainfuck_amd/csrc/merkle.hip:

```cpp
#include "blake2b_quad.hpp"
#include "merkle_core.hpp"
#include <vector>

#include "runtime.hpp"

namespace bfs {

constexpr int LEAF_THREADS = 64;

constexpr int LEAF_STAGE_WORDS = XFE_STREAM_WORDS * LEAF_THREADS;

__device__ __forceinline__ void xfe_leaves_wave(u64 c0, u64 c1, u64 c2, bool active, u64* stage , u64 h[8], const u64* midstates) {
    const u32 lane = threadIdx.x;
    const u32 k = active ? xfe_leaf_k(c0, c1, c2) : 0u;
    if (active && k == 0) merkle_leaf_xfe_zero(h, midstates);
    if (__ballot(k == 3) != 0) { if (k == 3) merkle_leaf_xfe_stream<3>(c0, c1, c2, stage + lane, LEAF_THREADS, h, midstates); }
    if (__ballot(k == 2) != 0) { if (k == 2) merkle_leaf_xfe_stream<2>(c0, c1, c2, stage + lane, LEAF_THREADS, h, midstates); }
    if (__ballot(k == 1) != 0) { if (k == 1) merkle_leaf_xfe_stream<1>(c0, c1, c2, stage + lane, LEAF_THREADS, h, midstates); }
}

__device__ __forceinline__ void xfe_leaves_wave_store(u64 c0, u64 c1, u64 c2, bool active, u64* stage, u64* leaf_digests, u64 i, const u64* midstates) {
    u64 d[8];
    xfe_leaves_wave(c0, c1, c2, active, stage, d, midstates);
    if (!active) return;
    u64* out = leaf_digests + i * 8;
#pragma unroll
    for (int j = 0; j < 8; ++j) out[j] = d[j];
}

__global__ void __launch_bounds__(LEAF_THREADS) merkle_leaves_xfe_kernel(const u64* limbs, u64 limb_stride, u64 n, u64* leaf_digests, const u64* midstates) {
    __shared__ u64 stage[LEAF_STAGE_WORDS];
    const u64 i = (u64)blockIdx.x * LEAF_THREADS + threadIdx.x;
    const bool active = i < n;
    u64 c0 = 0, c1 = 0, c2 = 0;
    if (active) { c0 = limbs[i]; c1 = limbs[limb_stride + i]; c2 = limbs[2 * limb_stride + i]; }
    xfe_leaves_wave_store(c0, c1, c2, active, stage, leaf_digests, i, midstates);
}

template <int K>
__global__ void __launch_bounds__(LEAF_THREADS) merkle_leaves_xfe_fold_kernel(FriFoldArgs f, u64* cw, u64 cw_stride, u64 n, u64* leaf_digests, const u64* midstates) {
    __shared__ u64 stage[LEAF_STAGE_WORDS];
    const u64 i = (u64)blockIdx.x * LEAF_THREADS + threadIdx.x;
    const bool active = i < n;
    u64 c0 = 0, c1 = 0, c2 = 0;
    if (active) {
        const Xfe r = fri_fold_point<K>(f, i);
        c0 = r.c[0];
        c1 = r.c[1];
        c2 = r.c[2];
        cw[i] = c0;
        cw[cw_stride + i] = c1;
        cw[2 * cw_stride + i] = c2;
    }
    xfe_leaves_wave_store(c0, c1, c2, active, stage, leaf_digests, i, midstates);
}

__global__ void __launch_bounds__(LEAF_THREADS) merkle_leaves_bfe_kernel(const u64* values, u64 n, u64* leaf_digests) {
    __shared__ u64 stage[BFE_LEAF_MAX_WORDS * LEAF_THREADS];
    const u64 i = (u64)blockIdx.x * LEAF_THREADS + threadIdx.x;
    if (i >= n) return;
    u64 d[8];
    merkle_leaf_bfe_body(values, i, stage + threadIdx.x, LEAF_THREADS, d);
    u64* out = leaf_digests + i * 8;
#pragma unroll
    for (int j = 0; j < 8; ++j) out[j] = d[j];
}

__global__ void blake2b_batch_kernel(const u64* data, const u64* offsets, const u32* lengths, u64 n, u64* digests) {
    const u64 i = (u64)blockIdx.x * blockDim.x + threadIdx.x;
    if (i >= n) return;
    u64 h[8];
    blake2b_staged<true>(data + offsets[i], 1, lengths[i], h);
    u64* out = digests + i * 8;
#pragma unroll
    for (int j = 0; j < 8; ++j) out[j] = h[j];
}

__global__ void merkle_parents_kernel(u64* nodes, u64 first, u64 count, u64 present_children) {
    const u64 t = (u64)blockIdx.x * blockDim.x + threadIdx.x;
    if (t >= count) return;
    const u64 k = first + t;
    const u64 c = 2 * t;
    int present = c + 1 < present_children ? 2 : (c < present_children ? 1 : 0);
    u64 out[8];
    merkle_parent_body(nodes + (2 * k) * 8, nodes + (2 * k + 1) * 8, present, out);
    u64* dst = nodes + k * 8;
#pragma unroll
    for (int j = 0; j < 8; ++j) dst[j] = out[j];
}

__global__ void __launch_bounds__(256) merkle_top_kernel(u64* nodes, u32 width, u64 present_children, u64* root_out, u64 seq) {
    __shared__ u64 lvl[512 * 8];
    const u32 t = threadIdx.x;
    for (u32 i = t; i < 2 * width * 8; i += 256) lvl[i] = nodes[(u64)2 * width * 8 + i];
    __syncthreads();
    u64 present = present_children;
    for (u32 w = width; w >= 1; w >>= 1) {
        u64 out[8];
        if (t < w) {
            const u64 c = 2 * (u64)t;
            int pr = c + 1 < present ? 2 : (c < present ? 1 : 0);
            merkle_parent_body(lvl + (2 * t) * 8, lvl + (2 * t + 1) * 8, pr, out);
        }
        __syncthreads();
        if (t < w) {
            u64* dst = nodes + ((u64)w + t) * 8;
#pragma unroll
            for (int j = 0; j < 8; ++j) { lvl[t * 8 + j] = out[j]; dst[j] = out[j]; }
            if (w == 1 && root_out != nullptr) {
#pragma unroll
                for (int j = 0; j < 8; ++j) __hip_atomic_store(root_out + j, out[j], __ATOMIC_RELAXED, __HIP_MEMORY_SCOPE_SYSTEM);
                __hip_atomic_store(root_out + 8, seq, __ATOMIC_RELEASE, __HIP_MEMORY_SCOPE_SYSTEM);
            }
        }
        __syncthreads();
        present = 2 * (u64)w;
    }
}


__global__ void __launch_bounds__(256) merkle_parents_quad_kernel(u64* nodes, u64 first, u64 count, u64 present_children) {
#if defined(__HIP_DEVICE_COMPILE__)
    __shared__ u64 msg[64 * 16];
    const u32 q = threadIdx.x >> 2, j = threadIdx.x & 3;
    const u64 t = (u64)blockIdx.x * 64 + q;
    const QuadLane ql = quad_lane(threadIdx.x);
    if (t < count) {
        const u64 k = first + t, c = 2 * t;
        const int present = c + 1 < present_children ? 2 : (c < present_children ? 1 : 0);
        const u64* child = nodes + (2 * k) * 8;
#pragma unroll
        for (int w = 0; w < 4; ++w) {
            const int idx = 4 * j + w;
            msg[q * 16 + idx] = (idx < 8 * present) ? child[idx] : 0;
        }
        u64 hl, hh;
        blake2b_init_quad(ql, hl, hh);
        blake2b_compress_quad(ql, hl, hh, msg + q * 16, (u64)(64 * present + 32 * (2 - present)), true);
        nodes[k * 8 + j] = hl;
        nodes[k * 8 + 4 + j] = hh;
    }
#endif
}

#if defined(__HIP_DEVICE_COMPILE__)
__device__ __forceinline__ void quad_parent(const QuadLane& ql, const u64* m, u64 bytes, u64& hl, u64& hh) {
    blake2b_init_quad(ql, hl, hh);
    blake2b_compress_quad(ql, hl, hh, m, bytes, true);
}
__device__ __forceinline__ void quad_parent_store(u32 j, u64 hl, u64 hh, u64* dst, u64* g) {
    dst[j] = hl;
    dst[4 + j] = hh;
    g[j] = hl;
    g[4 + j] = hh;
}

constexpr int QUAD_LEAF_WORDS = 48;

__device__ __forceinline__ void xfe_leaf_quad(u64 c0, u64 c1, u64 c2, u64* m, const QuadLane& ql, u32 j, const u64* midstates, u64& hl, u64& hh) {
    const u32 k = xfe_leaf_k(c0, c1, c2);
    if (k == 0) {
        hl = midstates[(size_t)2 * LEAF_MS_LEN * 8 + j];
        hh = midstates[(size_t)2 * LEAF_MS_LEN * 8 + 4 + j];
    } else {
        const u32 body = xfe_leaf_body_len(k, c0, c1, c2), total = body + 11;
        const u32 nblk = (total + 127) / 128;
        const u64* ms = midstates + ((size_t)(k == 1 ? 0 : 1) * LEAF_MS_LEN + body) * 8;
        hl = ms[j];
        hh = ms[4 + j];
        if (j == 0) {
            LeafWriter w;
            w.init(m, 1);
            encode_xfe_leaf_tail(w, k, c0, c1, c2);
            for (u32 x = w.wpos; x < (nblk - 1) * 16; ++x) m[x] = 0;
        }
        for (u32 b = 1; b < nblk; ++b) {
            const bool last = b + 1 == nblk;
            blake2b_compress_quad(ql, hl, hh, m + 16 * (b - 1), last ? (u64)total : (u64)(b + 1) * 128, last);
        }
    }
}
#endif

__global__ void __launch_bounds__(1024) merkle_top_quad_kernel(u64* nodes, u32 width, u64 present_children, u64* root_out, u64 seq) {
#if defined(__HIP_DEVICE_COMPILE__)
    __shared__ u64 bufA[512 * 8];
    __shared__ u64 bufB[256 * 8];
    const u32 tid = threadIdx.x, q = tid >> 2, j = tid & 3;
    const QuadLane ql = quad_lane(tid);
    for (u32 i = tid; i < 2 * width * 8; i += 1024) bufA[i] = nodes[(u64)2 * width * 8 + i];
    __syncthreads();
    u64* src = bufA;
    u64* dst = bufB;
    u64 present = present_children;
    for (u32 w = width; w >= 1; w >>= 1) {
        if (q < w) {
            const u64 c = 2 * (u64)q;
            const int pr = c + 1 < present ? 2 : (c < present ? 1 : 0);
            u64* m = src + q * 16;
            if (pr < 2) {
#pragma unroll
                for (int wd = 0; wd < 4; ++wd) { const int idx = 4 * j + wd; if (idx >= 8 * pr) m[idx] = 0; }
            }
            u64 hl, hh;
            quad_parent(ql, m, (u64)(64 * pr + 32 * (2 - pr)), hl, hh);
            quad_parent_store(j, hl, hh, dst + q * 8, nodes + ((u64)w + q) * 8);
            if (w == 1 && root_out != nullptr) {
                __hip_atomic_store(root_out + j, hl, __ATOMIC_RELAXED, __HIP_MEMORY_SCOPE_SYSTEM);
                __hip_atomic_store(root_out + 4 + j, hh, __ATOMIC_RELAXED, __HIP_MEMORY_SCOPE_SYSTEM);
            }
        }
        __syncthreads();
        u64* tmp = src; src = dst; dst = tmp;
        present = 2 * (u64)w;
    }
    if (tid == 0 && root_out != nullptr) {
        __threadfence_system();
        __hip_atomic_store(root_out + 8, seq, __ATOMIC_RELEASE, __HIP_MEMORY_SCOPE_SYSTEM);
    }
#endif
}

__global__ void __launch_bounds__(1024) merkle_subtree_quad_kernel(u64* nodes, u64 children) {
#if defined(__HIP_DEVICE_COMPILE__)
    __shared__ u64 bufA[512 * 8];
    __shared__ u64 bufB[256 * 8];
    const u32 tid = threadIdx.x, q = tid >> 2, j = tid & 3;
    const QuadLane ql = quad_lane(tid);
    const u64* in = nodes + (children + (u64)blockIdx.x * 512) * 8;
    for (u32 i = tid; i < 512 * 8; i += 1024) bufA[i] = in[i];
    __syncthreads();
    u64* src = bufA;
    u64* dst = bufB;
    u64 level = children >> 1;
    for (u32 w = 256; w >= 1; w >>= 1, level >>= 1) {
        if (q < w) {
            u64 hl, hh;
            quad_parent(ql, src + q * 16, 128, hl, hh);
            quad_parent_store(j, hl, hh, dst + q * 8, nodes + (level + (u64)blockIdx.x * w + q) * 8);
        }
        __syncthreads();
        u64* tmp = src; src = dst; dst = tmp;
    }
#endif
}

__global__ void __launch_bounds__(256) merkle_leaves_xfe_quad_kernel(const u64* limbs, u64 limb_stride, u64 n, u64* leaf_digests, const u64* midstates) {
#if defined(__HIP_DEVICE_COMPILE__)
    __shared__ u64 stage[64 * QUAD_LEAF_WORDS];
    const u32 q = threadIdx.x >> 2, j = threadIdx.x & 3;
    const u64 i = (u64)blockIdx.x * 64 + q;
    const QuadLane ql = quad_lane(threadIdx.x);
    if (i >= n) return;
    u64* m = stage + q * QUAD_LEAF_WORDS;
    const u64 c0 = limbs[i], c1 = limbs[limb_stride + i], c2 = limbs[2 * limb_stride + i];
    u64 hl, hh;
    xfe_leaf_quad(c0, c1, c2, m, ql, j, midstates, hl, hh);
    leaf_digests[i * 8 + j] = hl;
    leaf_digests[i * 8 + 4 + j] = hh;
#endif
}

constexpr u32 FRI_WG_LEAVES = 64;

template <int K>
__global__ void __launch_bounds__(4 * FRI_WG_LEAVES) fri_round_quad_kernel(FriFoldArgs f, u64* cw, u64 cw_stride, u64 n, u64* nodes, const u64* midstates,
                                                              u64* root_out, u64 seq) {
#if defined(__HIP_DEVICE_COMPILE__)
    __shared__ u64 stage[FRI_WG_LEAVES * QUAD_LEAF_WORDS];
    __shared__ u64 bufA[FRI_WG_LEAVES * 8];
    __shared__ u64 bufB[FRI_WG_LEAVES * 4];
    __shared__ u64 limbs[3 * FRI_WG_LEAVES];
    const u32 tid = threadIdx.x, q = tid >> 2, j = tid & 3;
    const QuadLane ql = quad_lane(tid);
    const u32 local = n < FRI_WG_LEAVES ? (u32)n : FRI_WG_LEAVES;
    const u64 first = (u64)blockIdx.x * FRI_WG_LEAVES;
    if (tid < local) {
        const u64 i = first + tid;
        u64 c0, c1, c2;
        if (f.in != nullptr) {
            const Xfe r = fri_fold_point<K>(f, i);
            c0 = r.c[0]; c1 = r.c[1]; c2 = r.c[2];
            cw[i] = c0; cw[cw_stride + i] = c1; cw[2 * cw_stride + i] = c2;
        } else {
            c0 = cw[i]; c1 = cw[cw_stride + i]; c2 = cw[2 * cw_stride + i];
        }
        limbs[tid] = c0; limbs[FRI_WG_LEAVES + tid] = c1; limbs[2 * FRI_WG_LEAVES + tid] = c2;
    }
    __syncthreads();
    if (q < local) {
        u64* m = stage + q * QUAD_LEAF_WORDS;
        const u64 c0 = limbs[q], c1 = limbs[FRI_WG_LEAVES + q], c2 = limbs[2 * FRI_WG_LEAVES + q];
        u64 hl, hh;
        xfe_leaf_quad(c0, c1, c2, m, ql, j, midstates, hl, hh);
        u64* g = nodes + (n + first + q) * 8;
        g[j] = hl; g[4 + j] = hh;
        bufA[q * 8 + j] = hl; bufA[q * 8 + 4 + j] = hh;
    }
    __syncthreads();
    u64* src = bufA;
    u64* dst = bufB;
    const u64 groups = n / local;
    const bool whole_tree = groups == 1;
    for (u32 w = local >> 1; w >= 1; w >>= 1) {
        if (q < w) {
            u64 hl, hh;
            quad_parent(ql, src + q * 16, 128, hl, hh);
            quad_parent_store(j, hl, hh, dst + q * 8, nodes + (groups * w + (u64)blockIdx.x * w + q) * 8);
            if (w == 1 && whole_tree && root_out != nullptr) {
                __hip_atomic_store(root_out + j, hl, __ATOMIC_RELAXED, __HIP_MEMORY_SCOPE_SYSTEM);
                __hip_atomic_store(root_out + 4 + j, hh, __ATOMIC_RELAXED, __HIP_MEMORY_SCOPE_SYSTEM);
            }
        }
        __syncthreads();
        u64* tmp = src; src = dst; dst = tmp;
    }
    if (tid == 0 && whole_tree && root_out != nullptr) {
        __threadfence_system();
        __hip_atomic_store(root_out + 8, seq, __ATOMIC_RELEASE, __HIP_MEMORY_SCOPE_SYSTEM);
    }
#endif
}

constexpr u64 QUAD_PARENTS_MAX = 8192;
constexpr u64 SUBTREE_PARENTS_MAX = 65536;
constexpr u64 QUAD_LEAVES_MAX = 8192;

int merkle_inner_launch(u64* d_nodes, u32 depth, u64 n_leaves, hipStream_t stream, u64* root_out, u64 seq) {
    if (depth == 0) return BFS_OK;
    u64 present = n_leaves;
    for (u32 lvl = depth; lvl-- > 0;) {
        const u64 count = 1ull << lvl;
        if (present >= 2 * count && count >= 512 && count <= SUBTREE_PARENTS_MAX) {
            hipLaunchKernelGGL(merkle_subtree_quad_kernel, dim3((u32)(count / 256)), dim3(1024), 0, stream, d_nodes, 2 * count);
            BFS_HIP(hipGetLastError());
            lvl -= 8;
            present = 2 * count;
            continue;
        }
        if (count <= 256) {
            hipLaunchKernelGGL(merkle_top_quad_kernel, dim3(1), dim3(1024), 0, stream, d_nodes, (u32)count, present, root_out, seq);
            BFS_HIP(hipGetLastError());
            return BFS_OK;
        }
        if (count <= QUAD_PARENTS_MAX)
            hipLaunchKernelGGL(merkle_parents_quad_kernel, dim3((u32)((count + 63) / 64)), dim3(256), 0, stream, d_nodes, count, count, present);
        else
            hipLaunchKernelGGL(merkle_parents_kernel, dim3((u32)((count + 255) / 256)), dim3(256), 0, stream, d_nodes, count, count, present);
        BFS_HIP(hipGetLastError());
        present = 2 * count;
    }
    return BFS_OK;
}

static int get_leaf_midstates(const u64** d_table) {
    if (cached_table_lookup(0x6D696473ULL, 1, 0, d_table)) return BFS_OK;
    std::vector<u64> host(LEAF_MS_WORDS);
    leaf_midstates(host.data());
    return cached_table(0x6D696473ULL, 1, 0, host.data(), host.size(), d_table);
}

int merkle_build_xfe_launch(const u64* d_limbs, u64 limb_stride, u64 n, u64* d_nodes, hipStream_t stream, u64* root_out, u64 seq) {
    if (n == 0) return BFS_OK;
    const u64* d_ms = nullptr;
    BFS_TRY(get_leaf_midstates(&d_ms));
    const u32 depth = tree_depth(n);
    const u64 npo2 = 1ull << depth;
    if (n <= QUAD_LEAVES_MAX)
        hipLaunchKernelGGL(merkle_leaves_xfe_quad_kernel, dim3((u32)((n + 63) / 64)), dim3(256), 0, stream, d_limbs, limb_stride, n, d_nodes + npo2 * 8, d_ms);
    else
        hipLaunchKernelGGL(merkle_leaves_xfe_kernel, dim3((u32)((n + LEAF_THREADS - 1) / LEAF_THREADS)), dim3(LEAF_THREADS), 0, stream,
                           d_limbs, limb_stride, n, d_nodes + npo2 * 8, d_ms);
    BFS_HIP(hipGetLastError());
    return merkle_inner_launch(d_nodes, depth, n, stream, root_out, seq);
}

int fri_round_fused_launch(const FriFoldArgs& fold, u64* d_cw, u64 cw_stride, u64 n, u64* d_nodes, hipStream_t stream, u64* root_out, u64 seq) {
    if (n < 2 || n > FRI_FUSED_MAX || (n & (n - 1))) { set_error("internal: fused FRI round on %llu elements", (unsigned long long)n); return BFS_ERR_BAD_ARG; }
    const u64* d_ms = nullptr;
    BFS_TRY(get_leaf_midstates(&d_ms));
    const u32 groups = (u32)(n <= FRI_WG_LEAVES ? 1 : n / FRI_WG_LEAVES);
    const dim3 grid(groups), block(4 * FRI_WG_LEAVES);
    BFS_TRY(with_fold_factor(fold.in == nullptr ? 1u : fold.log2_folding, [&](auto k) -> int {
        hipLaunchKernelGGL(fri_round_quad_kernel<decltype(k)::value>, grid, block, 0, stream, fold, d_cw, cw_stride, n, d_nodes, d_ms, root_out, seq);
        BFS_HIP(hipGetLastError());
        return BFS_OK;
    }));
    if (groups == 1) return BFS_OK;
    return merkle_inner_launch(d_nodes, tree_depth(groups), groups, stream, root_out, seq);
}

int merkle_build_xfe_fold_launch(const FriFoldArgs& fold, u64* d_cw, u64 cw_stride, u64 n, u64* d_nodes, hipStream_t stream, u64* root_out, u64 seq) {
    if (fold.in == nullptr || n <= QUAD_LEAVES_MAX) { set_error("internal: fused fold + leaves on %llu elements", (unsigned long long)n); return BFS_ERR_BAD_ARG; }
    const u64* d_ms = nullptr;
    BFS_TRY(get_leaf_midstates(&d_ms));
    const u32 depth = tree_depth(n);
    const u64 npo2 = 1ull << depth;
    const dim3 grid((u32)((n + LEAF_THREADS - 1) / LEAF_THREADS)), block(LEAF_THREADS);
    BFS_TRY(with_fold_factor(fold.log2_folding, [&](auto k) -> int {
        hipLaunchKernelGGL(merkle_leaves_xfe_fold_kernel<decltype(k)::value>, grid, block, 0, stream, fold, d_cw, cw_stride, n, d_nodes + npo2 * 8, d_ms);
        BFS_HIP(hipGetLastError());
        return BFS_OK;
    }));
    return merkle_inner_launch(d_nodes, depth, n, stream, root_out, seq);
}

int merkle_build_bfe_launch(const u64* d_values, u64 n, u64* d_nodes, hipStream_t stream) {
    if (n == 0) return BFS_OK;
    const u32 depth = tree_depth(n);
    const u64 npo2 = 1ull << depth;
    hipLaunchKernelGGL(merkle_leaves_bfe_kernel, dim3((u32)((n + LEAF_THREADS - 1) / LEAF_THREADS)), dim3(LEAF_THREADS), 0, stream,
                       d_values, n, d_nodes + npo2 * 8);
    BFS_HIP(hipGetLastError());
    return merkle_inner_launch(d_nodes, depth, n, stream);
}

int merkle_build_bytes_launch(const u64* d_data, const u64* d_offsets, const u32* d_lengths, u64 n, u64* d_nodes, hipStream_t stream) {
    if (n == 0) return BFS_OK;
    const u32 depth = tree_depth(n);
    const u64 npo2 = 1ull << depth;
    hipLaunchKernelGGL(blake2b_batch_kernel, dim3((u32)((n + 63) / 64)), dim3(64), 0, stream, d_data, d_offsets, d_lengths, n, d_nodes + npo2 * 8);
    BFS_HIP(hipGetLastError());
    return merkle_inner_launch(d_nodes, depth, n, stream);
}

}
```

stark_brainfuck_amd/csrc/runtime.hpp:

```cpp
#pragma once
#include <hip/hip_runtime.h>
#include <stddef.h>
#include <stdint.h>

#include <type_traits>

#include "ntt_plan.hpp"

namespace bfs {

void set_error(const char* fmt, ...) __attribute__((format(printf, 1, 2)));
const char* last_error();

#define BFS_HIP(expr)                                                                                   \
    do {                                                                                                \
        hipError_t e_ = (expr);                                                                         \
        if (e_ != hipSuccess) {                                                                         \
            ::bfs::set_error("%s failed: %s (%s:%d)", #expr, hipGetErrorString(e_), __FILE__, __LINE__); \
            return BFS_ERR_HIP;                                                                         \
        }                                                                                               \
    } while (0)

#define BFS_TRY(expr)            \
    do {                         \
        int rc_ = (expr);        \
        if (rc_) return rc_;     \
    } while (0)

int workspace(int slot, size_t bytes, hipStream_t stream, void** out);
int workspace_release(int slot, hipStream_t stream);
bool workspace_peek(int slot, hipStream_t stream, void** ptr, size_t* bytes);

static const hipStream_t NO_STREAM = (hipStream_t)(uintptr_t)-1;
int device_alloc(size_t bytes, hipStream_t stream, void** out);
int device_release(void* ptr, hipStream_t stream);
int device_pool_trim();
void device_pool_stats(size_t* live_bytes, size_t* cached_bytes);
int host_alloc(size_t bytes, void** out);
int host_release(void* ptr);

int copy_h2d(void* d, const void* h, size_t bytes, hipStream_t stream);
int copy_d2h(void* h, const void* d, size_t bytes, hipStream_t stream);

int stream_retire(hipStream_t stream);

int cached_table(uint64_t key_a, uint64_t key_b, uint64_t key_c, const u64* host, size_t count, const u64** d_out);
bool cached_table_lookup(uint64_t key_a, uint64_t key_b, uint64_t key_c, const u64** d_out);

struct FriFoldArgs {
    const u64* in;
    u64 in_stride, half;
    Xfe alpha[3];
    u64 scal[7];
    const u64* winv_lo;
    const u64* winv_hi;
    u32 lo_bits, round_shift;
    u32 log2_folding;
};
inline void fri_fold_constants(FriFoldArgs& f, u32 k, u64 n, const Xfe& alpha, u64 offset, u64 omega) {
    f.log2_folding = k;
    f.half = n >> k;
    f.alpha[0] = alpha;
    for (u32 j = 1; j < 3; ++j) f.alpha[j] = j < k ? xfe_mul(f.alpha[j - 1], f.alpha[j - 1]) : Xfe{{0, 0, 0}};
    u64 gj = gl_mul(gl_inv(2), gl_inv(offset));
    u64 zj = k > 1 ? gl_pow(gl_inv(omega), f.half) : 1;
    u32 off = 0;
    for (u32 j = 0; j < k; ++j) {
        const u32 h = 1u << (k - 1 - j);
        u64 z = 1;
        for (u32 m = 0; m < h; ++m) { f.scal[off + m] = gl_mul(gj, z); z = gl_mul(z, zj); }
        off += h;
        gj = gl_mul(gl_mul(gj, gj), 2);
        zj = gl_sqr(zj);
    }
    for (; off < 7; ++off) f.scal[off] = 0;
}

BFS_HD u64 gl_half(u64 x) { return (x >> 1) + ((x & 1) ? 0x7FFFFFFF80000001ULL : 0); }

template <int K>
BFS_HD Xfe fri_fold_point(const FriFoldArgs& f, u64 i) {
    constexpr int A = 1 << K;
    Xfe v[A];
    BFS_UNROLL
    for (int m = 0; m < A; ++m) {
        const u64 at = (u64)m * f.half + i;
        v[m] = Xfe{{f.in[at], f.in[f.in_stride + at], f.in[2 * f.in_stride + at]}};
    }
    u64 w = tw_pow(f.winv_lo, f.winv_hi, f.lo_bits, i << f.round_shift);
    int off = 0;
    BFS_UNROLL
    for (int j = 0; j < K; ++j) {
        const int h = 1 << (K - 1 - j);
        BFS_UNROLL
        for (int m = 0; m < h; ++m) {
            const u64 s = gl_mul(f.scal[off + m], w);
            const Xfe beta = xfe_scale(f.alpha[j], s);
            const Xfe sum = xfe_add(v[m], v[m + h]), diff = xfe_sub(v[m], v[m + h]);
            const Xfe prod = xfe_mul(beta, diff);
            v[m] = Xfe{{gl_add(gl_half(sum.c[0]), prod.c[0]), gl_add(gl_half(sum.c[1]), prod.c[1]), gl_add(gl_half(sum.c[2]), prod.c[2])}};
        }
        off += h;
        if (j + 1 < K) w = gl_sqr(w);
    }
    return v[0];
}
template <class Fn>
inline int with_fold_factor(u32 log2_folding, Fn&& fn) {
    switch (log2_folding) {
    case 1: return fn(std::integral_constant<int, 1>());
    case 2: return fn(std::integral_constant<int, 2>());
    case 3: return fn(std::integral_constant<int, 3>());
    default: set_error("internal: fold by 2^%u", log2_folding); return BFS_ERR_BAD_ARG;
    }
}
inline u32 tree_depth(u64 n) {
    u32 depth = 0;
    while ((1ull << depth) < n) ++depth;
    return depth;
}
constexpr u64 FRI_FUSED_MAX = 16384;
int merkle_build_xfe_fold_launch(const FriFoldArgs& fold, u64* d_cw, u64 cw_stride, u64 n, u64* d_nodes, hipStream_t stream, u64* root_out, u64 seq);
int fri_round_fused_launch(const FriFoldArgs& fold, u64* d_cw, u64 cw_stride, u64 n, u64* d_nodes, hipStream_t stream, u64* root_out, u64 seq);

struct NttCall {
    const u64* in;
    u64 n_in, in_stride;
    u64* out;
    u64 out_stride;
    u32 batch;
    u64 root, shift, post_scale;
    u32 streaming;
    hipStream_t stream;
};
constexpr u64 NTT_STREAMING_BYTES = 128ull << 20;
int ntt_launch(const u64* d_in, u64 n_in, u64 in_stride, u64* d_out, u64 out_stride, u32 log_n, u32 batch, u64 root,
               u64 shift, u64 post_scale, hipStream_t stream);
int ntt_run_steps(const NttCall& c, const NttPlan& p, u64* mid, u32 first, u32 last);
int ntt_power_tables(u64 root, u32 log_n, const u64** lo, const u64** hi, u32* lo_bits);
constexpr int NTT_ROUTE_CANDIDATES = 3;
constexpr int NTT_ROUTE_DIRECT = -1;
enum class NttRouteMode { Remembered, Auto, Forced };
struct NttEnv {
    NttRouteMode route_mode;
    int forced_route;
    bool probe_log;
    int force_streaming;
    bool allow_expand;
    bool plan_log;
};
const NttEnv& ntt_env();

constexpr int NTT_ROUTE_SLOT0 = 16;
int ntt_route(const NttCall& c, const NttPlan& p, int* route);
int ntt_route_probe_info(float* us, int* route, unsigned long long* probes);
int ntt_tune(const u64* d_in, u64 in_stride, u64* d_out, u64 out_stride, u32 log_n, u32 batch, u64 root, hipStream_t stream, int* route_out);
size_t ntt_route_forget_range(const void* lo, size_t bytes, bool may_free);
void ntt_route_trim();

int mul_pointwise_launch(const u64* a, const u64* b, u64* out, u64 n, hipStream_t stream);
int batch_inverse_launch(const u64* in, u64* out, u64 n, hipStream_t stream);
int scale_launch(const u64* in, u64* out, u64 n, u64 stride, u32 batch, u64 factor, hipStream_t stream);
int xfe_mul_pointwise_launch(const u64* a, u64 a_stride, const u64* b, u64 b_stride, u64* out, u64 out_stride, u64 n, hipStream_t stream);
int xfe_batch_inverse_launch(const u64* in, u64 in_stride, u64* out, u64 out_stride, u64 n, hipStream_t stream);

int merkle_inner_launch(u64* d_nodes, u32 depth, u64 n_leaves, hipStream_t stream, u64* root_out = nullptr, u64 seq = 0);
int merkle_build_xfe_launch(const u64* d_limbs, u64 limb_stride, u64 n, u64* d_nodes, hipStream_t stream, u64* root_out = nullptr, u64 seq = 0);
int merkle_build_bfe_launch(const u64* d_values, u64 n, u64* d_nodes, hipStream_t stream);
int merkle_build_bytes_launch(const u64* d_data, const u64* d_offsets, const u32* d_lengths, u64 n, u64* d_nodes, hipStream_t stream);

int coset_tree_launch(const FriFoldArgs* fold, u64* d_cw, u64 cw_stride, u64 q, u32 log2_coset, u64* d_nodes, hipStream_t stream, u64* not_mine,
                      u64 token, u64* root_out, u64 seq);
int coset_tree_rows(const u64* d_cw, u64 cw_stride, u64 q, u32 log2_coset, u64* d_nodes, unsigned char h_root[64], hipStream_t stream);

constexpr u64 POW_DEFAULT_WINDOW = 1ULL << 24;
int pow_search(const u64 seed[4], u32 bits, u64 first, u64 count, u64* nonce, bool* found, hipStream_t stream);

struct PinnedLease {
    void* host = nullptr;
    void* dev = nullptr;
    int get(size_t need) {
        BFS_TRY(host_alloc(need < 4096 ? 4096 : need, &host));
        BFS_HIP(hipHostGetDevicePointer(&dev, host, 0));
        return BFS_OK;
    }
    ~PinnedLease() { if (host) (void)host_release(host); }
    PinnedLease() = default;
    PinnedLease(const PinnedLease&) = delete;
    PinnedLease& operator=(const PinnedLease&) = delete;
};

}
```

Measured before the change: 103.0 billion.

## Pre-launch armed FRI round kernels that spin-wait on host-served challenges

Small FRI rounds (fused one-launch and coset paths) can now be launched before their folding challenge is known. Their kernels poll a pinned host mailbox slot until the host writes alpha, or until the host calls them off or a time budget runs out. This aims to hide kernel launch latency between the host transcript step and the next round. It adds per-round mailboxes, a give-up and fallback path, and the risk of GPU time spent busy-waiting; the metric is NTT throughput, which this path likely does not touch.

```diff
diff --git a/include/bfstark.h b/include/bfstark.h
--- a/include/bfstark.h
+++ b/include/bfstark.h
@@ -191,6 +191,7 @@
                          uint32_t expansion_factor, uint32_t log2_folding, int coset_leaves, uint32_t num_colinearity_tests,
                          uint64_t* h_top_level_indices, void* stream);
 void bfs_fri_last_timing(double out[6]);
+void bfs_fri_last_armed(uint32_t out[3]);
 uint32_t bfs_fri_session_rounds(void* session);
 uint64_t bfs_fri_session_round_leaves(void* session, uint32_t round);
 int bfs_fri_session_round(void* session, uint32_t round, const uint64_t** d_codeword, uint64_t* length, uint64_t* limb_stride,
diff --git a/stark_brainfuck_amd/_lib.py b/stark_brainfuck_amd/_lib.py
--- a/stark_brainfuck_amd/_lib.py
+++ b/stark_brainfuck_amd/_lib.py
@@ -123,6 +123,7 @@
     "bfs_fri_prove": (ci, [vp, vp, u64, u32, u64, u64, u32, u32, ctypes.POINTER(u64), vp]),
     "bfs_fri_prove_folded": (ci, [vp, vp, u64, u32, u64, u64, u32, u32, u32, ctypes.POINTER(u64), vp]),
     "bfs_fri_last_timing": (None, [ctypes.POINTER(ctypes.c_double)]),
+    "bfs_fri_last_armed": (None, [ctypes.POINTER(u32)]),
     "bfs_fri_session_rounds": (u32, [vp]),
     "bfs_fri_session_round": (ci, [vp, u32, ctypes.POINTER(vp), ctypes.POINTER(u64), ctypes.POINTER(u64), ctypes.POINTER(vp), vp]),
     "bfs_selftest_field": (ci, [u32, ctypes.POINTER(u64)]),
diff --git a/stark_brainfuck_amd/csrc/coset.hip b/stark_brainfuck_amd/csrc/coset.hip
--- a/stark_brainfuck_amd/csrc/coset.hip
+++ b/stark_brainfuck_amd/csrc/coset.hip
@@ -3,16 +3,20 @@
 
 #include "../../include/bfstark.h"
 #include "coset_core.hpp"
+#include "fri_armed.hpp"
 #include "runtime.hpp"
 
 namespace bfs {
 
 constexpr u32 COSET_THREADS = 64;
 
-template <int K, int A>
+template <int K, int A, bool ARMED>
 __global__ void __launch_bounds__(COSET_THREADS) coset_leaves_kernel(FriFoldArgs f, u64* cw, u64 cw_stride, u64 q, u64* leaf_digests,
-                                                                     const u64* block0_states, u64* not_mine, u64 token) {
+                                                                     const u64* block0_states, u64* not_mine, u64 token, FriArmed armed) {
     typedef CosetShape<A> Shape;
+#if defined(__HIP_DEVICE_COMPILE__)
+    if constexpr (ARMED) { if (!fri_armed_wait(armed, f)) return; }
+#endif
     __shared__ __attribute__((aligned(16))) unsigned char blk[COSET_LANE_BYTES * COSET_THREADS];
     unsigned char* const buf = blk + COSET_LANE_BYTES * threadIdx.x;
     const u64 c = (u64)blockIdx.x * COSET_THREADS + threadIdx.x;
@@ -91,22 +95,25 @@
 }
 
 template <int KF, int A = 1 << KF>
-static int coset_leaves_launch_a(const FriFoldArgs* fold, u64* d_cw, u64 cw_stride, u64 q, u64* d_leaf_digests, hipStream_t stream, u64* not_mine, u64 token) {
+static int coset_leaves_launch_a(const FriFoldArgs* fold, u64* d_cw, u64 cw_stride, u64 q, u64* d_leaf_digests, hipStream_t stream, u64* not_mine, u64 token,
+                                 const FriArmed* armed) {
     const u64* d_states = nullptr;
     BFS_TRY(coset_block0_states<A>(&d_states));
     const dim3 grid((u32)((q + COSET_THREADS - 1) / COSET_THREADS)), block(COSET_THREADS);
-    if (fold != nullptr) hipLaunchKernelGGL((coset_leaves_kernel<KF, A>), grid, block, 0, stream, *fold, d_cw, cw_stride, q, d_leaf_digests, d_states, not_mine, token);
-    else hipLaunchKernelGGL((coset_leaves_kernel<0, A>), grid, block, 0, stream, FriFoldArgs{}, d_cw, cw_stride, q, d_leaf_digests, d_states, not_mine, token);
+    if (armed != nullptr) hipLaunchKernelGGL((coset_leaves_kernel<KF, A, true>), grid, block, 0, stream, *fold, d_cw, cw_stride, q, d_leaf_digests, d_states, not_mine, token, *armed);
+    else if (fold != nullptr) hipLaunchKernelGGL((coset_leaves_kernel<KF, A, false>), grid, block, 0, stream, *fold, d_cw, cw_stride, q, d_leaf_digests, d_states, not_mine, token, FriArmed{});
+    else hipLaunchKernelGGL((coset_leaves_kernel<0, A, false>), grid, block, 0, stream, FriFoldArgs{}, d_cw, cw_stride, q, d_leaf_digests, d_states, not_mine, token, FriArmed{});
     BFS_HIP(hipGetLastError());
     return BFS_OK;
 }
 
 int coset_tree_launch(const FriFoldArgs* fold, u64* d_cw, u64 cw_stride, u64 q, u32 log2_coset, u64* d_nodes, hipStream_t stream, u64* not_mine,
-                      u64 token, u64* root_out, u64 seq) {
+                      u64 token, u64* root_out, u64 seq, const FriArmed* armed) {
+    if (armed != nullptr && (fold == nullptr || armed->slot == nullptr)) { set_error("internal: armed coset tree without a fold"); return BFS_ERR_BAD_ARG; }
     if (q == 0 || (q & (q - 1))) { set_error("internal: coset tree over %llu leaves", (unsigned long long)q); return BFS_ERR_BAD_ARG; }
     if (fold != nullptr && (fold->log2_folding != log2_coset || fold->half != (q << log2_coset))) { set_error("internal: coset tree and fold disagree"); return BFS_ERR_BAD_ARG; }
     BFS_TRY(with_fold_factor(log2_coset, [&](auto k) -> int {
-        return coset_leaves_launch_a<decltype(k)::value>(fold, d_cw, cw_stride, q, d_nodes + q * 8, stream, not_mine, token);
+        return coset_leaves_launch_a<decltype(k)::value>(fold, d_cw, cw_stride, q, d_nodes + q * 8, stream, not_mine, token, armed);
     }));
     return merkle_inner_launch(d_nodes, tree_depth(q), q, stream, root_out, seq);
 }
diff --git a/stark_brainfuck_amd/csrc/fri.hip b/stark_brainfuck_amd/csrc/fri.hip
--- a/stark_brainfuck_amd/csrc/fri.hip
+++ b/stark_brainfuck_amd/csrc/fri.hip
@@ -1,6 +1,7 @@
 #include <algorithm>
 #include <chrono>
 #include <map>
+#include <thread>
 #include <unordered_map>
 #include <vector>
 
@@ -57,6 +58,7 @@
 }
 
 static thread_local double g_fri_timing[8] = {0, 0, 0, 0, 0, 0, 0, 0};
+static thread_local uint32_t g_fri_armed[3] = {0, 0, 0};
 static inline double now_ms() { return std::chrono::duration<double, std::milli>(std::chrono::steady_clock::now().time_since_epoch()).count(); }
 
 enum class TreePath : unsigned char {
@@ -74,17 +76,65 @@
     u64 leaves = 0;
     u64* nodes = nullptr;
     TreePath path = TreePath::Codeword;
+    bool armed = false;
     unsigned char root[64];
 };
 
+constexpr u32 FRI_ARMED_CUS_PER_GROUP = 8;
+constexpr u32 FRI_ARMED_BUDGET_US = 500;
+struct FriArmedEnv {
+    bool on = true;
+    u64 max_groups = 0, budget_us = FRI_ARMED_BUDGET_US;
+    long withhold = -1;
+    FriArmedEnv() {
+        if (const char* e = getenv("BFS_FRI_ARMED")) on = atoi(e) != 0;
+        if (const char* e = getenv("BFS_FRI_ARMED_MAX_GROUPS")) max_groups = strtoull(e, nullptr, 10);
+        if (const char* e = getenv("BFS_FRI_ARMED_BUDGET_US")) budget_us = strtoull(e, nullptr, 10);
+        if (const char* e = getenv("BFS_FRI_ARMED_WITHHOLD")) withhold = atol(e);
+    }
+};
+static int fri_armed_device(u64* compute_units, u64* ticks_per_us) {
+    struct Dev { u64 cus = 0, ticks = 0; };
+    static Dev devs[64];
+    int dev = 0;
+    BFS_HIP(hipGetDevice(&dev));
+    Dev local, &d = dev >= 0 && dev < 64 ? devs[dev] : local;
+    if (__atomic_load_n(&d.ticks, __ATOMIC_ACQUIRE) == 0) {
+        int cus = 0, khz = 0;
+        BFS_HIP(hipDeviceGetAttribute(&cus, hipDeviceAttributeMultiprocessorCount, dev));
+        BFS_HIP(hipDeviceGetAttribute(&khz, hipDeviceAttributeWallClockRate, dev));
+        if (cus <= 0 || khz < 1000) { set_error("device %d reports %d compute units and a wall clock of %d kHz", dev, cus, khz); return BFS_ERR_HIP; }
+        d.cus = (u64)cus;
+        __atomic_store_n(&d.ticks, (u64)khz / 1000, __ATOMIC_RELEASE);
+    }
+    *compute_units = d.cus;
+    *ticks_per_us = d.ticks;
+    return BFS_OK;
+}
+
+struct ChallengeBox {
+    u64* host = nullptr;
+    u64* dev = nullptr;
+    void serve(u32 round, const Xfe& alpha, u64 seq) {
+        u64* slot = host + (size_t)round * FRI_SLOT_WORDS;
+        const u64 tag = (u64)(u32)seq << 32;
+        for (int c = 0; c < 3; ++c) {
+            __atomic_store_n(slot + 2 * c, tag | (u32)alpha.c[c], __ATOMIC_RELAXED);
+            __atomic_store_n(slot + 2 * c + 1, tag | (alpha.c[c] >> 32), __ATOMIC_RELAXED);
+        }
+    }
+    void call_off(u32 round, u64 seq) { __atomic_store_n(host + (size_t)round * FRI_SLOT_WORDS, (u64)~(u32)seq << 32, __ATOMIC_RELAXED); }
+};
+
 struct RootMailbox {
+    static constexpr u32 SLOTS = 64;
     u64* host = nullptr;
     u64* dev = nullptr;
     u64 seq = 0;
     int init() {
         if (host) return BFS_OK;
-        BFS_TRY(host_alloc(16 * sizeof(u64), (void**)&host));
-        memset(host, 0, 16 * sizeof(u64));
+        BFS_TRY(host_alloc(SLOTS * (16 + FRI_SLOT_WORDS) * sizeof(u64), (void**)&host));
+        memset(host, 0, SLOTS * (16 + FRI_SLOT_WORDS) * sizeof(u64));
         BFS_HIP(hipHostGetDevicePointer((void**)&dev, host, 0));
         return BFS_OK;
     }
@@ -96,6 +146,12 @@
     void* block = nullptr;
     bool use_workspace = false;
     RootMailbox mailbox;
+    ChallengeBox box;
+    bool arming = false;
+    u64 armed_budget = 0;
+    long armed_withhold = -1;
+    u32 pending_round = 0;
+    u64 pending_seq = 0;
     u32 log_n = 0;
     u32 log2_folding = 1;
     bool coset_leaves = false;
@@ -153,6 +209,7 @@
     const u32 R = fri_num_rounds(N, expansion, k);
     if (k > 1 && R < 2) { set_error("cannot fold by %u with less than one fold", 1u << k); return BFS_ERR_BAD_ARG; }
     if (R < 1) { set_error("cannot do FRI with less than one round"); return BFS_ERR_BAD_ARG; }
+    if (R > RootMailbox::SLOTS) { set_error("internal: %u rounds", R); return BFS_ERR_BAD_ARG; }
     if (gl_pow(omega, N) != 1 || (log_n && gl_pow(omega, N / 2) == 1)) {
         set_error("error in commit: omega does not have the right order!");
         return BFS_ERR_NOT_ROOT;
@@ -165,6 +222,19 @@
         set_error("the round-0 tree handed to the session has %llu leaves, this session's has %llu", (unsigned long long)(S.round0_leaves ? S.round0_leaves : N),
                   (unsigned long long)(coset ? N >> k : N));
         return BFS_ERR_BAD_ARG;
+    }
+    const FriArmedEnv env;
+    u64 armed_groups = 0, ticks_per_us = 0;
+    S.arming = false;
+    S.pending_round = 0;
+    if (env.on) {
+        hipStreamCaptureStatus capture = hipStreamCaptureStatusActive;
+        if (hipStreamIsCapturing(stream, &capture) != hipSuccess) { (void)hipGetLastError(); capture = hipStreamCaptureStatusActive; }
+        if (capture == hipStreamCaptureStatusNone) {
+            BFS_TRY(fri_armed_device(&armed_groups, &ticks_per_us));
+            armed_groups /= FRI_ARMED_CUS_PER_GROUP;
+            if (env.max_groups) armed_groups = env.max_groups;
+        }
     }
     size_t words = 0;
     for (u32 r = 0; r < R; ++r) {
@@ -178,7 +248,10 @@
                   : fr.length <= FRI_FUSED_MAX ? TreePath::OneLaunch
                   : r >= 1                 ? TreePath::FoldInLeaves
                                            : TreePath::Codeword;
-        words += (size_t)16 * fr.leaves + (r ? (size_t)3 * fr.length : 0);
+        const u64 groups = (fr.leaves + 63) / 64;
+        fr.armed = r >= 1 && (fr.path == TreePath::OneLaunch || fr.path == TreePath::Coset) && groups <= armed_groups;
+        S.arming = S.arming || fr.armed;
+        words +=(size_t)16 * fr.leaves + (r ? (size_t)3 * fr.length : 0);
     }
     u64* p = nullptr;
     if (S.use_workspace) {
@@ -197,16 +270,28 @@
         if (r == 0) { fr.cw = d_cw; fr.stride = stride; }
         else { fr.cw = p; fr.stride = fr.length; p += 3 * fr.length; }
     }
-    return S.mailbox.init();
-}
-
-static int launch_round_tree(FriSession& S, u32 r, const FriFoldArgs& fold, hipStream_t stream, u64* seq) {
+    BFS_TRY(S.mailbox.init());
+    if (S.arming) {
+        S.box.host = S.mailbox.host + RootMailbox::SLOTS * 16;
+        S.box.dev = S.mailbox.dev + RootMailbox::SLOTS * 16;
+        memset(S.box.host, 0, (size_t)R * FRI_SLOT_WORDS * sizeof(u64));
+        S.armed_budget = env.budget_us * ticks_per_us;
+        S.armed_withhold = env.withhold;
+    }
+    return BFS_OK;
+}
+
+static int launch_round_tree(FriSession& S, u32 r, const FriFoldArgs& fold, hipStream_t stream, u64* seq, bool armed = false) {
     FriRound& fr = S.rounds[r];
     const bool folds = fold.in != nullptr;
     u64* const cw = (u64*)fr.cw;
-    u64* const box = S.mailbox.dev;
+    u64* const box = S.mailbox.dev + (size_t)16 * r;
     *seq = 0;
     if (folds != (r >= 1)) { set_error("internal: round %u of the plan and its fold disagree", r); return BFS_ERR_BAD_ARG; }
+    if (armed && !fr.armed) { set_error("internal: round %u of the plan is not one to arm", r); return BFS_ERR_BAD_ARG; }
+    FriArmed arm{};
+    if (armed) arm = FriArmed{S.box.dev + (size_t)r * FRI_SLOT_WORDS, S.mailbox.seq + 1, box + 10, S.armed_budget};
+    const FriArmed* const armp = armed ? &arm : nullptr;
     switch (fr.path) {
     case TreePath::Borrowed:
         fr.nodes = (u64*)S.round0_nodes;
@@ -217,10 +302,10 @@
         return merkle_build_xfe_launch(fr.cw, fr.stride, fr.length, fr.nodes, stream);
     case TreePath::Coset:
         *seq = ++S.mailbox.seq;
-        return coset_tree_launch(folds ? &fold : nullptr, cw, fr.stride, fr.leaves, S.log2_folding, fr.nodes, stream, box + 9, *seq, box, *seq);
+        return coset_tree_launch(folds ? &fold : nullptr, cw, fr.stride, fr.leaves, S.log2_folding, fr.nodes, stream, box + 9, *seq, box, *seq, armp);
     case TreePath::OneLaunch:
         *seq = ++S.mailbox.seq;
-        return fri_round_fused_launch(fold, cw, fr.stride, fr.length, fr.nodes, stream, box, *seq);
+        return fri_round_fused_launch(fold, cw, fr.stride, fr.length, fr.nodes, stream, box, *seq, armp);
     case TreePath::FoldInLeaves:
         *seq = ++S.mailbox.seq;
         return merkle_build_xfe_fold_launch(fold, cw, fr.stride, fr.length, fr.nodes, stream, box, *seq);
@@ -232,8 +317,8 @@
     return BFS_ERR_BAD_ARG;
 }
 
-int fri_commit(FriSession& S, rp::Transcript& ps, const u64* d_cw, u64 stride, u32 log_n, u64 offset, u64 omega,
-               u32 expansion, hipStream_t stream) {
+static int fri_commit_rounds(FriSession& S, rp::Transcript& ps, const u64* d_cw, u64 stride, u32 log_n, u64 offset, u64 omega,
+                             u32 expansion, hipStream_t stream) {
     const double t_begin = now_ms();
     BFS_TRY(plan_rounds(S, d_cw, stride, log_n, omega, expansion, stream));
     const u32 k = S.log2_folding;
@@ -243,6 +328,8 @@
     BFS_TRY(ntt_power_tables(gl_inv(omega), log_n, &winv_lo, &winv_hi, &lo_bits));
     u64 g = offset, w = omega;
     FriFoldArgs fold{};
+    u64 armed_seq = 0;
+    g_fri_armed[0] = g_fri_armed[1] = g_fri_armed[2] = 0;
     rp::Transcript::Lookahead look;
     static const bool lookahead_on = getenv("BFS_FRI_LOOKAHEAD") == nullptr || atoi(getenv("BFS_FRI_LOOKAHEAD")) != 0;
     static const bool trace = getenv("BFS_FRI_TRACE") != nullptr;
@@ -261,7 +348,7 @@
         const double t_round = trace ? now_ms() : 0;
         double t_launched = 0, t_absorbed = 0, t_root = 0;
         rp::Transcript::Speculation speculation;
-        auto await_root = [&](u64 seq) -> int {
+        auto await_prepare = [&]() {
             if (trace) t_launched = now_ms();
             if (r >= 1) begin_lookahead();
             if (r + 1 < R) {
@@ -269,23 +356,69 @@
                 else if (!looking) { ps.speculate(speculation); speculating = true; }
             }
             if (trace) t_absorbed = now_ms();
-            volatile u64* flag = S.mailbox.host + 8;
+        };
+        auto await_root = [&](u64 seq, bool armed, bool* unserved) -> int {
+            const u64* const box = S.mailbox.host + (size_t)16 * r;
+            const u64* flag = box + 8;
+            const u64* gave_up = box + 10;
             u64 spins = 0;
+            *unserved = false;
             while (__atomic_load_n(flag, __ATOMIC_ACQUIRE) != seq) {
+                if (armed && __atomic_load_n(gave_up, __ATOMIC_ACQUIRE) == seq) { *unserved = true; return BFS_OK; }
                 if (++spins > (1ull << 22)) {
+                    if (S.pending_round != 0) {
+                        const hipError_t state = hipStreamQuery(stream);
+                        if (state == hipErrorNotReady) { std::this_thread::sleep_for(std::chrono::microseconds(20)); continue; }
+                        BFS_HIP(state);
+                    }
                     BFS_HIP(hipStreamSynchronize(stream));
+                    if (armed && __atomic_load_n(gave_up, __ATOMIC_ACQUIRE) == seq) { *unserved = true; return BFS_OK; }
                     if (__atomic_load_n(flag, __ATOMIC_ACQUIRE) != seq) { set_error("root mailbox was not written"); return BFS_ERR_HIP; }
                     break;
                 }
             }
-            memcpy(fr.root, S.mailbox.host, 64);
+            if (armed && __atomic_load_n(gave_up, __ATOMIC_ACQUIRE) == seq) { *unserved = true; return BFS_OK; }
+            memcpy(fr.root, box, 64);
             return BFS_OK;
         };
+        auto call_off_pending = [&]() {
+            if (S.pending_round == 0) return;
+            S.box.call_off(S.pending_round, S.pending_seq);
+            S.pending_round = 0;
+        };
         u64 seq = 0;
-        BFS_TRY(launch_round_tree(S, r, fold, stream, &seq));
+        const bool was_armed = armed_seq != 0;
+        if (was_armed) seq = armed_seq;
+        else BFS_TRY(launch_round_tree(S, r, fold, stream, &seq));
+        armed_seq = 0;
+        FriFoldArgs next{};
+        if (r + 1 < R) {
+            next.in = fr.cw; next.in_stride = fr.stride;
+            next.winv_lo = winv_lo; next.winv_hi = winv_hi; next.lo_bits = lo_bits; next.round_shift = k * r;
+            fri_fold_domain_constants(next, k, fr.length, g, w);
+            if (S.arming && S.rounds[r + 1].armed) {
+                BFS_TRY(launch_round_tree(S, r + 1, next, stream, &armed_seq, true));
+                S.pending_round = r + 1; S.pending_seq = armed_seq;
+                ++g_fri_armed[0];
+            }
+        }
+        const char* how = was_armed ? "  armed, served" : "";
         if (seq != 0) {
-            BFS_TRY(await_root(seq));
-            if (fr.path == TreePath::Coset && __atomic_load_n(S.mailbox.host + 9, __ATOMIC_ACQUIRE) == seq) {
+            bool unserved = false;
+            await_prepare();
+            BFS_TRY(await_root(seq, was_armed, &unserved));
+            if (unserved) {
+                call_off_pending();
+                armed_seq = 0;
+                S.arming = false;
+                ++g_fri_armed[2];
+                how = "  armed, unserved: launched again";
+                BFS_HIP(hipStreamSynchronize(stream));
+                BFS_TRY(launch_round_tree(S, r, fold, stream, &seq));
+                BFS_TRY(await_root(seq, false, &unserved));
+            } else if (was_armed) ++g_fri_armed[1];
+            if (fr.path == TreePath::Coset && __atomic_load_n(S.mailbox.host + (size_t)16 * r + 9, __ATOMIC_ACQUIRE) == seq) {
+                if (armed_seq != 0) { call_off_pending(); armed_seq = 0; }
                 BFS_TRY(coset_tree_rows(fr.cw, fr.stride, fr.leaves, k, fr.nodes, fr.root, stream));
             }
         } else if (fr.path == TreePath::SingleElement) {
@@ -297,15 +430,17 @@
         if (speculating) ps.resolve(speculation, fr.root, seed, 32);
         else if (r > 0 && looking) { ps.lookahead_next(look, fr.root, r + 1 < R ? seed : nullptr, 32); have_seed = r + 1 < R; }
         else if (r > 0) ps.objects.push_back(rp::mk_bytes(fr.root, 64));
+        if (r + 1 < R) {
+            if (!speculating && !have_seed) ps.fiat_shamir(ps.objects.size(), seed, 32);
+            fri_fold_challenge_constants(next.alpha, k, rp::sample_xfe(seed, 32));
+            if (armed_seq != 0 && S.armed_withhold != (long)(r + 1)) S.box.serve(r + 1, next.alpha[0], armed_seq);
+            if (armed_seq != 0) S.pending_round = 0;
+            fold = next;
+            for (u32 j = 0; j < k; ++j) { g = gl_sqr(g); w = gl_sqr(w); }
+        }
         if (trace)
-            fprintf(stderr, "fri round %2u  n %8llu  launch %6.1f us  absorb %6.1f us  wait %6.1f us  finish %6.1f us\n", r, (unsigned long long)fr.length,
-                    1e3 * (t_launched - t_round), 1e3 * (t_absorbed - t_launched), 1e3 * (t_root - t_absorbed), 1e3 * (now_ms() - t_root));
-        if (r == R - 1) break;
-        if (!speculating && !have_seed) ps.fiat_shamir(ps.objects.size(), seed, 32);
-        fold.in = fr.cw; fold.in_stride = fr.stride;
-        fold.winv_lo = winv_lo; fold.winv_hi = winv_hi; fold.lo_bits = lo_bits; fold.round_shift = k * r;
-        fri_fold_constants(fold, k, fr.length, rp::sample_xfe(seed, 32), g, w);
-        for (u32 j = 0; j < k; ++j) { g = gl_sqr(g); w = gl_sqr(w); }
+            fprintf(stderr, "fri round %2u  n %8llu  launch %6.1f us  absorb %6.1f us  wait %6.1f us  finish %6.1f us%s\n", r, (unsigned long long)fr.length,
+                    1e3 * (t_launched - t_round), 1e3 * (t_absorbed - t_launched), 1e3 * (t_root - t_absorbed), 1e3 * (now_ms() - t_root), how);
     }
     g_fri_timing[0] = now_ms() - t_begin;
     FriRound& last = S.rounds[R - 1];
@@ -327,6 +462,17 @@
     ps.objects.push_back(rp::mk_list(items));
     g_fri_timing[1] = now_ms() - t_begin - g_fri_timing[0];
     return BFS_OK;
+}
+
+int fri_commit(FriSession& S, rp::Transcript& ps, const u64* d_cw, u64 stride, u32 log_n, u64 offset, u64 omega,
+               u32 expansion, hipStream_t stream) {
+    const int rc = fri_commit_rounds(S, ps, d_cw, stride, log_n, offset, omega, expansion, stream);
+    if (rc != BFS_OK && S.pending_round != 0) {
+        S.box.call_off(S.pending_round, S.pending_seq);
+        S.pending_round = 0;
+        (void)hipStreamSynchronize(stream);
+    }
+    return rc;
 }
 
 static int sample_indices(const unsigned char seed[32], u64 size, u64 reduced_size, u32 number, std::vector<u64>& out) {
@@ -750,6 +896,8 @@
 
 void bfs_fri_last_timing(double out[6]) { for (int i = 0; i < 6; ++i) out[i] = g_fri_timing[i]; }
 
+void bfs_fri_last_armed(uint32_t out[3]) { for (int i = 0; i < 3; ++i) out[i] = g_fri_armed[i]; }
+
 uint32_t bfs_fri_session_rounds(void* session) { return (uint32_t)((FriSession*)session)->rounds.size(); }
 
 int bfs_fri_session_round(void* session, uint32_t r, const uint64_t** d_codeword, uint64_t* length, uint64_t* limb_stride,
diff --git a/stark_brainfuck_amd/csrc/fri_armed.hpp b/stark_brainfuck_amd/csrc/fri_armed.hpp
--- /dev/null
+++ b/stark_brainfuck_amd/csrc/fri_armed.hpp
@@ -0,0 +1,44 @@
+#pragma once
+#include "runtime.hpp"
+
+namespace bfs {
+
+#if defined(__HIP_DEVICE_COMPILE__)
+__device__ __forceinline__ u64 fri_uniform(u64 v) {
+    const u32 lo = (u32)__builtin_amdgcn_readfirstlane((int)(u32)v), hi = (u32)__builtin_amdgcn_readfirstlane((int)(u32)(v >> 32));
+    return ((u64)hi << 32) | lo;
+}
+
+__device__ __forceinline__ bool fri_armed_wait(const FriArmed& a, FriFoldArgs& f) {
+    __shared__ u32 box[8];
+    if (threadIdx.x < 64) {
+        const u32 lane = threadIdx.x, tag = (u32)a.seq;
+        const u64 t0 = wall_clock64();
+        u64 word = 0;
+        bool served;
+        for (;;) {
+            if (lane < 6) word = __hip_atomic_load(a.slot + lane, __ATOMIC_RELAXED, __HIP_MEMORY_SCOPE_SYSTEM);
+            const u32 got = (u32)(word >> 32);
+            served = __ballot(lane < 6 && got == tag) == 0x3Full;
+            const bool off = __ballot(lane < 6 && got == ~tag) != 0;
+            if (served || off || wall_clock64() - t0 > a.budget) break;
+            __builtin_amdgcn_s_sleep(4);
+        }
+        if (served) { if (lane < 6) box[lane] = (u32)word; }
+        else if (lane == 0) __hip_atomic_store(a.unserved, a.seq, __ATOMIC_RELAXED, __HIP_MEMORY_SCOPE_SYSTEM);
+        if (lane == 0) box[6] = served;
+    }
+    __syncthreads();
+    if (box[6] == 0) return false;
+    Xfe alpha;
+#pragma unroll
+    for (int c = 0; c < 3; ++c) alpha.c[c] = fri_uniform(((u64)box[2 * c + 1] << 32) | box[2 * c]);
+    fri_fold_challenge_constants(f.alpha, f.log2_folding, alpha);
+#pragma unroll
+    for (int j = 1; j < 3; ++j)
+        for (int c = 0; c < 3; ++c) f.alpha[j].c[c] = fri_uniform(f.alpha[j].c[c]);
+    return true;
+}
+#endif
+
+}
diff --git a/stark_brainfuck_amd/csrc/merkle.hip b/stark_brainfuck_amd/csrc/merkle.hip
--- a/stark_brainfuck_amd/csrc/merkle.hip
+++ b/stark_brainfuck_amd/csrc/merkle.hip
@@ -1,4 +1,5 @@
 #include "blake2b_quad.hpp"
+#include "fri_armed.hpp"
 #include "merkle_core.hpp"
 #include <vector>
 
@@ -263,10 +264,11 @@
 
 constexpr u32 FRI_WG_LEAVES = 64;
 
-template <int K>
+template <int K, bool ARMED>
 __global__ void __launch_bounds__(4 * FRI_WG_LEAVES) fri_round_quad_kernel(FriFoldArgs f, u64* cw, u64 cw_stride, u64 n, u64* nodes, const u64* midstates,
-                                                              u64* root_out, u64 seq) {
-#if defined(__HIP_DEVICE_COMPILE__)
+                                                              u64* root_out, u64 seq, FriArmed armed) {
+#if defined(__HIP_DEVICE_COMPILE__)
+    if constexpr (ARMED) { if (!fri_armed_wait(armed, f)) return; }
     __shared__ u64 stage[FRI_WG_LEAVES * QUAD_LEAF_WORDS];
     __shared__ u64 bufA[FRI_WG_LEAVES * 8];
     __shared__ u64 bufB[FRI_WG_LEAVES * 4];
@@ -375,14 +377,17 @@
     return merkle_inner_launch(d_nodes, depth, n, stream, root_out, seq);
 }
 
-int fri_round_fused_launch(const FriFoldArgs& fold, u64* d_cw, u64 cw_stride, u64 n, u64* d_nodes, hipStream_t stream, u64* root_out, u64 seq) {
+int fri_round_fused_launch(const FriFoldArgs& fold, u64* d_cw, u64 cw_stride, u64 n, u64* d_nodes, hipStream_t stream, u64* root_out, u64 seq, const FriArmed* armed) {
+    if (armed != nullptr && (fold.in == nullptr || armed->slot == nullptr)) { set_error("internal: armed FRI round without a fold"); return BFS_ERR_BAD_ARG; }
     if (n < 2 || n > FRI_FUSED_MAX || (n & (n - 1))) { set_error("internal: fused FRI round on %llu elements", (unsigned long long)n); return BFS_ERR_BAD_ARG; }
     const u64* d_ms = nullptr;
     BFS_TRY(get_leaf_midstates(&d_ms));
     const u32 groups = (u32)(n <= FRI_WG_LEAVES ? 1 : n / FRI_WG_LEAVES);
     const dim3 grid(groups), block(4 * FRI_WG_LEAVES);
     BFS_TRY(with_fold_factor(fold.in == nullptr ? 1u : fold.log2_folding, [&](auto k) -> int {
-        hipLaunchKernelGGL(fri_round_quad_kernel<decltype(k)::value>, grid, block, 0, stream, fold, d_cw, cw_stride, n, d_nodes, d_ms, root_out, seq);
+        constexpr int K = decltype(k)::value;
+        if (armed != nullptr) hipLaunchKernelGGL((fri_round_quad_kernel<K, true>), grid, block, 0, stream, fold, d_cw, cw_stride, n, d_nodes, d_ms, root_out, seq, *armed);
+        else hipLaunchKernelGGL((fri_round_quad_kernel<K, false>), grid, block, 0, stream, fold, d_cw, cw_stride, n, d_nodes, d_ms, root_out, seq, FriArmed{});
         BFS_HIP(hipGetLastError());
         return BFS_OK;
     }));
diff --git a/stark_brainfuck_amd/csrc/runtime.hpp b/stark_brainfuck_amd/csrc/runtime.hpp
--- a/stark_brainfuck_amd/csrc/runtime.hpp
+++ b/stark_brainfuck_amd/csrc/runtime.hpp
@@ -57,11 +57,9 @@
     u32 lo_bits, round_shift;
     u32 log2_folding;
 };
-inline void fri_fold_constants(FriFoldArgs& f, u32 k, u64 n, const Xfe& alpha, u64 offset, u64 omega) {
+inline void fri_fold_domain_constants(FriFoldArgs& f, u32 k, u64 n, u64 offset, u64 omega) {
     f.log2_folding = k;
     f.half = n >> k;
-    f.alpha[0] = alpha;
-    for (u32 j = 1; j < 3; ++j) f.alpha[j] = j < k ? xfe_mul(f.alpha[j - 1], f.alpha[j - 1]) : Xfe{{0, 0, 0}};
     u64 gj = gl_mul(gl_inv(2), gl_inv(offset));
     u64 zj = k > 1 ? gl_pow(gl_inv(omega), f.half) : 1;
     u32 off = 0;
@@ -75,6 +73,22 @@
     }
     for (; off < 7; ++off) f.scal[off] = 0;
 }
+BFS_HD void fri_fold_challenge_constants(Xfe out[3], u32 k, const Xfe& alpha) {
+    out[0] = alpha;
+    for (u32 j = 1; j < 3; ++j) out[j] = j < k ? xfe_mul(out[j - 1], out[j - 1]) : Xfe{{0, 0, 0}};
+}
+inline void fri_fold_constants(FriFoldArgs& f, u32 k, u64 n, const Xfe& alpha, u64 offset, u64 omega) {
+    fri_fold_domain_constants(f, k, n, offset, omega);
+    fri_fold_challenge_constants(f.alpha, k, alpha);
+}
+
+constexpr u32 FRI_SLOT_WORDS = 8;
+struct FriArmed {
+    const u64* slot;
+    u64 seq;
+    u64* unserved;
+    u64 budget;
+};
 
 BFS_HD u64 gl_half(u64 x) { return (x >> 1) + ((x & 1) ? 0x7FFFFFFF80000001ULL : 0); }
 
@@ -121,7 +135,8 @@
 }
 constexpr u64 FRI_FUSED_MAX = 16384;
 int merkle_build_xfe_fold_launch(const FriFoldArgs& fold, u64* d_cw, u64 cw_stride, u64 n, u64* d_nodes, hipStream_t stream, u64* root_out, u64 seq);
-int fri_round_fused_launch(const FriFoldArgs& fold, u64* d_cw, u64 cw_stride, u64 n, u64* d_nodes, hipStream_t stream, u64* root_out, u64 seq);
+int fri_round_fused_launch(const FriFoldArgs& fold, u64* d_cw, u64 cw_stride, u64 n, u64* d_nodes, hipStream_t stream, u64* root_out, u64 seq,
+                           const FriArmed* armed = nullptr);
 
 struct NttCall {
     const u64* in;
@@ -170,7 +185,7 @@
 int merkle_build_bytes_launch(const u64* d_data, const u64* d_offsets, const u32* d_lengths, u64 n, u64* d_nodes, hipStream_t stream);
 
 int coset_tree_launch(const FriFoldArgs* fold, u64* d_cw, u64 cw_stride, u64 q, u32 log2_coset, u64* d_nodes, hipStream_t stream, u64* not_mine,
-                      u64 token, u64* root_out, u64 seq);
+                      u64 token, u64* root_out, u64 seq, const FriArmed* armed = nullptr);
 int coset_tree_rows(const u64* d_cw, u64 cw_stride, u64 q, u32 log2_coset, u64* d_nodes, unsigned char h_root[64], hipStream_t stream);
 
 constexpr u64 POW_DEFAULT_WINDOW = 1ULL << 24;
```

Result: no change. 103.0 billion (-0.0%).
